# sail-sg/EditAnything

Measured on NVIDIA H100. Metric: 512x512 50-step SAM+ControlNet-inpaint images/sec; fused ControlNetx2+UNet+CFG+DDIM step ms, higher is better.
Workload: dtype fp16 storage / fp32 accumulate

## Files before the change

editanything_b200/csrc/ea_common.cuh:

```cuda
#pragma once
#include <cuda.h>
#include <cuda_fp16.h>
#include <cuda_bf16.h>
#include <cuda_runtime.h>
#include <stdint.h>
#include "ea_wgmma.cuh"

#ifdef EA_USE_BF16
typedef __nv_bfloat16 ea_half;
typedef __nv_bfloat162 ea_half2;
#define EA_TMAP_DTYPE CU_TENSOR_MAP_DATA_TYPE_BFLOAT16
__device__ __forceinline__ float ea_h2f(ea_half h) { return __bfloat162float(h); }
__device__ __forceinline__ ea_half ea_f2h(float f) { return __float2bfloat16_rn(f); }
__device__ __forceinline__ uint32_t ea_pack2(float a, float b) {
  __nv_bfloat162 v = __floats2bfloat162_rn(a, b);
  return *reinterpret_cast<uint32_t*>(&v);
}
__device__ __forceinline__ float2 ea_unpack2(uint32_t u) {
  __nv_bfloat162 v = *reinterpret_cast<__nv_bfloat162*>(&u);
  return __bfloat1622float2(v);
}
#else
typedef __half ea_half;
typedef __half2 ea_half2;
#define EA_TMAP_DTYPE CU_TENSOR_MAP_DATA_TYPE_FLOAT16
__device__ __forceinline__ float ea_h2f(ea_half h) { return __half2float(h); }
__device__ __forceinline__ ea_half ea_f2h(float f) { return __float2half_rn(f); }
__device__ __forceinline__ uint32_t ea_pack2(float a, float b) {
  __half2 v = __floats2half2_rn(a, b);
  return *reinterpret_cast<uint32_t*>(&v);
}
__device__ __forceinline__ float2 ea_unpack2(uint32_t u) {
  __half2 v = *reinterpret_cast<__half2*>(&u);
  return __half22float2(v);
}
#endif

namespace ea {

__device__ __forceinline__ uint32_t smem_u32(const void* p) {
  return static_cast<uint32_t>(__cvta_generic_to_shared(p));
}

__device__ __forceinline__ bool elect_one() {
  uint32_t pred = 0;
  asm volatile(
      "{\n\t.reg .pred P;\n\t"
      "elect.sync _|P, 0xffffffff;\n\t"
      "selp.b32 %0, 1, 0, P;\n\t}\n"
      : "=r"(pred));
  return pred != 0;
}

__device__ __forceinline__ void mbar_init(uint64_t* bar, uint32_t count) {
  asm volatile("mbarrier.init.shared::cta.b64 [%0], %1;" ::"r"(smem_u32(bar)), "r"(count));
}
__device__ __forceinline__ void fence_mbar_init() {
  asm volatile("fence.mbarrier_init.release.cluster;" ::: "memory");
}
__device__ __forceinline__ void fence_proxy_async() {
  asm volatile("fence.proxy.async.shared::cta;" ::: "memory");
}
__device__ __forceinline__ void mbar_expect_tx(uint64_t* bar, uint32_t bytes) {
  asm volatile("mbarrier.arrive.expect_tx.shared::cta.b64 _, [%0], %1;" ::"r"(smem_u32(bar)),
               "r"(bytes)
               : "memory");
}
__device__ __forceinline__ void mbar_arrive(uint64_t* bar) {
  asm volatile("mbarrier.arrive.shared::cta.b64 _, [%0];" ::"r"(smem_u32(bar)) : "memory");
}
__device__ __forceinline__ bool mbar_try_wait(uint64_t* bar, uint32_t parity) {
  uint32_t ok;
  asm volatile(
      "{\n\t.reg .pred P;\n\t"
      "mbarrier.try_wait.parity.shared::cta.b64 P, [%1], %2;\n\t"
      "selp.b32 %0, 1, 0, P;\n\t}\n"
      : "=r"(ok)
      : "r"(smem_u32(bar)), "r"(parity)
      : "memory");
  return ok != 0;
}
__device__ __forceinline__ void mbar_wait(uint64_t* bar, uint32_t parity) {
  uint32_t spins = 0;
  while (!mbar_try_wait(bar, parity)) {
    if (++spins > (1u << 28)) { asm volatile("trap;"); }
  }
}

__device__ __forceinline__ void tma_prefetch_desc(const CUtensorMap* m) {
  asm volatile("prefetch.tensormap [%0];" ::"l"(reinterpret_cast<uint64_t>(m)) : "memory");
}
__device__ __forceinline__ void tma_prefetch_l2_2d(const CUtensorMap* m, int c0, int c1) {
  asm volatile("cp.async.bulk.prefetch.tensor.2d.L2.global.tile [%0, {%1, %2}];" ::"l"(
                   reinterpret_cast<uint64_t>(m)),
               "r"(c0), "r"(c1)
               : "memory");
}
__device__ __forceinline__ void tma_load_2d(void* smem, const CUtensorMap* m, uint64_t* bar, int c0,
                                            int c1) {
  asm volatile(
      "cp.async.bulk.tensor.2d.shared::cluster.global.mbarrier::complete_tx::bytes [%0], [%1, {%3, "
      "%4}], [%2];" ::"r"(smem_u32(smem)),
      "l"(reinterpret_cast<uint64_t>(m)), "r"(smem_u32(bar)), "r"(c0), "r"(c1)
      : "memory");
}
__device__ __forceinline__ void tma_load_2d_hint(void* smem, const CUtensorMap* m, uint64_t* bar, int c0,
                                                 int c1, uint64_t policy) {
  if (policy == 0ull) {
    tma_load_2d(smem, m, bar, c0, c1);
    return;
  }
  asm volatile(
      "cp.async.bulk.tensor.2d.shared::cluster.global.mbarrier::complete_tx::bytes.L2::cache_hint [%0], [%1, {%3, "
      "%4}], [%2], %5;" ::"r"(smem_u32(smem)),
      "l"(reinterpret_cast<uint64_t>(m)), "r"(smem_u32(bar)), "r"(c0), "r"(c1), "l"(policy)
      : "memory");
}
__device__ __forceinline__ void tma_load_3d(void* smem, const CUtensorMap* m, uint64_t* bar, int c0,
                                            int c1, int c2) {
  asm volatile(
      "cp.async.bulk.tensor.3d.shared::cluster.global.mbarrier::complete_tx::bytes [%0], [%1, {%3, "
      "%4, %5}], [%2];" ::"r"(smem_u32(smem)),
      "l"(reinterpret_cast<uint64_t>(m)), "r"(smem_u32(bar)), "r"(c0), "r"(c1), "r"(c2)
      : "memory");
}
__device__ __forceinline__ void tma_load_4d(void* smem, const CUtensorMap* m, uint64_t* bar, int c0,
                                            int c1, int c2, int c3) {
  asm volatile(
      "cp.async.bulk.tensor.4d.shared::cluster.global.mbarrier::complete_tx::bytes [%0], [%1, {%3, "
      "%4, %5, %6}], [%2];" ::"r"(smem_u32(smem)),
      "l"(reinterpret_cast<uint64_t>(m)), "r"(smem_u32(bar)), "r"(c0), "r"(c1), "r"(c2), "r"(c3)
      : "memory");
}

__device__ __forceinline__ void wgmma_fence() { asm volatile("wgmma.fence.sync.aligned;" ::: "memory"); }
__device__ __forceinline__ void wgmma_commit() { asm volatile("wgmma.commit_group.sync.aligned;" ::: "memory"); }
template <int N>
__device__ __forceinline__ void wgmma_wait() {
  asm volatile("wgmma.wait_group.sync.aligned %0;" ::"n"(N) : "memory");
}
template <int R>
__device__ __forceinline__ void wgmma_fence_regs(float (&d)[R]) {
#pragma unroll
  for (int i = 0; i < R; ++i) asm volatile("" : "+f"(d[i])::"memory");
}

__device__ __forceinline__ uint64_t gmma_desc_k_sw128(uint32_t saddr, uint32_t sbo_bytes) {
  uint64_t d = 0;
  d |= (uint64_t)((saddr >> 4) & 0x3FFF);
  d |= (uint64_t)1 << 16;
  d |= (uint64_t)((sbo_bytes >> 4) & 0x3FFF) << 32;
  d |= (uint64_t)1 << 62;
  return d;
}
__device__ __forceinline__ uint64_t gmma_desc_mn_sw128(uint32_t saddr, uint32_t lbo_bytes,
                                                       uint32_t sbo_bytes) {
  uint64_t d = 0;
  d |= (uint64_t)((saddr >> 4) & 0x3FFF);
  d |= (uint64_t)((lbo_bytes >> 4) & 0x3FFF) << 16;
  d |= (uint64_t)((sbo_bytes >> 4) & 0x3FFF) << 32;
  d |= (uint64_t)1 << 62;
  return d;
}

__device__ __forceinline__ void pdl_wait() { asm volatile("griddepcontrol.wait;" ::: "memory"); }
__device__ __forceinline__ void pdl_launch_dependents() {
  asm volatile("griddepcontrol.launch_dependents;" ::: "memory");
}

__device__ __forceinline__ float mufu_ex2(float x) {
  float y;
  asm("ex2.approx.ftz.f32 %0, %1;" : "=f"(y) : "f"(x));
  return y;
}
__device__ __forceinline__ float mufu_rcp(float x) {
  float y;
  asm("rcp.approx.ftz.f32 %0, %1;" : "=f"(y) : "f"(x));
  return y;
}
__device__ __forceinline__ float silu_f(float x) {
  return x * mufu_rcp(1.0f + mufu_ex2(x * -1.4426950408889634f));
}
__device__ __forceinline__ float gelu_erf_f(float x) {
  const float z = fabsf(x) * 0.70710678118654752f;
  const float t = mufu_rcp(fmaf(0.3275911f, z, 1.0f));
  float poly = fmaf(1.061405429f, t, -1.453152027f);
  poly = fmaf(poly, t, 1.421413741f);
  poly = fmaf(poly, t, -0.284496736f);
  poly = fmaf(poly, t, 0.254829592f);
  const float e = fmaf(-poly * t, mufu_ex2(z * z * -1.4426950408889634f), 1.0f);
  return 0.5f * x * (1.0f + copysignf(e, x));
}
__device__ __forceinline__ float warp_sum(float v) {
#pragma unroll
  for (int o = 16; o > 0; o >>= 1) v += __shfl_xor_sync(0xffffffffu, v, o);
  return v;
}
__device__ __forceinline__ float warp_max(float v) {
#pragma unroll
  for (int o = 16; o > 0; o >>= 1) v = fmaxf(v, __shfl_xor_sync(0xffffffffu, v, o));
  return v;
}

}
```

editanything_b200/csrc/ea_gemm.cu:

```cuda
#include "ea_common.cuh"
#include "ea_internal.h"

namespace ea {

static constexpr int BM = 128;
static constexpr int BK = 64;
static constexpr int GEMM_THREADS = 288;
static constexpr int W_TMA = 8;
static constexpr int EPI_WARPS = 8, EPI_THREADS = 256;
static constexpr int GEMM_SMEM_RING = 216 * 1024;
__host__ __device__ constexpr int gemm_epi_bytes(int bn) { return BM * (bn + 4) * 4 + 2 * 4096 * EPI_WARPS; }
__host__ __device__ constexpr int gemm_region_bytes(int bn, int stages) {
  return stages * (BM * BK * 2 + bn * BK * 2) > gemm_epi_bytes(bn) ? stages * (BM * BK * 2 + bn * BK * 2)
                                                                    : gemm_epi_bytes(bn);
}

struct GemmKParams {
  int M, N;
  int mode;
  int nkb_main;
  int nkb_extra;
  int cin_blocks;
  int BN, stages;
  int H, W, Bsz;
  int bw, bh, bn;
  int tiles_w, tiles_h;
  const float* bias;
  const float* rowvec;
  int rows_per_batch;
  int rowvec_ld;
  const ea_half* residual;
  long long ldr;
  ea_half* out;
  long long ldo;
  ea_half* out2;
  long long ldo2;
  float* out_f32;
  int act;
  float out_scale;
  int accumulate;
  int splits;
  int kb_per_split;
  int no_spin;
  float* ws;
  int* cnt;
  float2* rowstats_out;
  const float2* ln_stats;
  const float* ln_g;
  int ln_parts;
  float ln_inv_c, ln_eps;
  const float* row_scale;
  const char* pf[EA_GEMM_MAX_PREFETCH];
  long long pf_bytes[EA_GEMM_MAX_PREFETCH];
  int pf_ctas;
  unsigned long long b_policy;
};

static constexpr int GEMM_MAX_GROUPS = 3;
struct GemmGroup {
  CUtensorMap tmA0, tmA1, tmA2, tmA3, tmAx, tmB;
  GemmKParams p;
};
template <int NG>
struct GemmLaunch {
  GemmGroup g[NG];
};

__device__ __forceinline__ void tile_origin(const GemmKParams& p, int tm, int& n0, int& h0,
                                            int& w0) {
  int per_blk = p.tiles_w * p.tiles_h;
  int nb = tm / per_blk;
  int r = tm - nb * per_blk;
  int th = r / p.tiles_w;
  n0 = nb * p.bn;
  h0 = th * p.bh;
  w0 = (r - th * p.tiles_w) * p.bw;
}

struct RowInfo {
  long long m;
  bool ok;
  int batch;
};

__device__ __forceinline__ RowInfo row_info(const GemmKParams& p, int tm, int r) {
  RowInfo ri;
  if (p.mode == EA_GEMM_LINEAR) {
    ri.m = (long long)tm * BM + r;
    ri.ok = ri.m < p.M;
    ri.batch = p.rows_per_batch > 0 ? (int)(ri.m / p.rows_per_batch) : 0;
  } else {
    int n0, h0, w0;
    tile_origin(p, tm, n0, h0, w0);
    int dn = r / (p.bw * p.bh);
    int rr = r - dn * (p.bw * p.bh);
    int dh = rr / p.bw;
    int dw = rr - dh * p.bw;
    int n = n0 + dn, h = h0 + dh, w = w0 + dw;
    ri.ok = (n < p.Bsz) && (h < p.H) && (w < p.W);
    ri.m = ((long long)n * p.H + h) * p.W + w;
    ri.batch = n;
  }
  return ri;
}

__device__ __forceinline__ void epi_bar_sync() { asm volatile("bar.sync 1, 256;" ::: "memory"); }

__device__ __forceinline__ int ld_acquire_gpu(const int* p) {
  int v;
  asm volatile("ld.acquire.gpu.global.s32 %0, [%1];" : "=r"(v) : "l"(p) : "memory");
  return v;
}

__device__ __forceinline__ void l2_prefetch_hint(const GemmKParams& p, int cta, int lane, int lane0) {
  if (cta >= p.pf_ctas || lane < lane0) return;
  const int nl = 32 - lane0;
#pragma unroll 1
  for (int i = 0; i < EA_GEMM_MAX_PREFETCH; ++i) {
    if (p.pf[i] == nullptr) continue;
    const long long nlines = p.pf_bytes[i] >> 7;
    const char* base = p.pf[i];
#pragma unroll 4
    for (long long c = (long long)cta * nl + (lane - lane0); c < nlines; c += (long long)p.pf_ctas * nl)
      asm volatile("prefetch.global.L2 [%0];" ::"l"(base + (c << 7)));
  }
}

__device__ __forceinline__ void ln_row_stats(const GemmKParams& p, long long m, float& ln_r, float& ln_nm) {
  float s = 0.f, q = 0.f;
  const float2* base = p.ln_stats + m;
  for (int j0 = 0; j0 < p.ln_parts; j0 += 16) {
    float2 v[16];
#pragma unroll
    for (int u = 0; u < 16; ++u)
      v[u] = (j0 + u < p.ln_parts) ? __ldcg(base + (size_t)(j0 + u) * p.M) : make_float2(0.f, 0.f);
#pragma unroll
    for (int u = 0; u < 16; ++u) {
      s += v[u].x;
      q += v[u].y;
    }
  }
  const float mu = s * p.ln_inv_c;
  ln_r = rsqrtf(fmaxf(q * p.ln_inv_c - mu * mu, 0.f) + p.ln_eps);
  ln_nm = -ln_r * mu;
}

__device__ __noinline__ float act_call(float x, int act) {
  return act == EA_ACT_SILU ? silu_f(x) : gelu_erf_f(x);
}

__device__ __forceinline__ void stage_put32(uint4* stg, int lane, int half, const uint4 (&o)[4]) {
#pragma unroll
  for (int q = 0; q < 4; ++q) stg[lane * 8 + ((half * 4 + q) ^ (lane & 7))] = o[q];
}
__device__ __forceinline__ void stage_flush(const uint4* stg, int lane, ea_half* out, long long ldo,
                                            ea_half* out2, long long ldo2, long long m_mine, bool ok_mine,
                                            int col0, int pieces, int n_limit, long long lin_m0, int M) {
  __syncwarp();
  const int piece = lane & 7, rsub = lane >> 3;
  const int col = col0 + piece * 8;
  const bool col_ok = piece < pieces && col < n_limit;
  uint4 val[8];
#pragma unroll
  for (int i = 0; i < 8; ++i) {
    const int row = i * 4 + rsub;
    val[i] = stg[row * 8 + (piece ^ (row & 7))];
  }
  if (lin_m0 >= 0) {
    const long long m0 = lin_m0 + rsub;
    ea_half* ptr = out + m0 * ldo + col;
    ea_half* ptr2 = out2 ? out2 + m0 * ldo2 + col : nullptr;
    const long long step = 4 * ldo, step2 = 4 * ldo2;
#pragma unroll
    for (int i = 0; i < 8; ++i) {
      if (col_ok && m0 + 4 * i < M) {
        *reinterpret_cast<uint4*>(ptr) = val[i];
        if (ptr2) *reinterpret_cast<uint4*>(ptr2) = val[i];
      }
      ptr += step;
      if (ptr2) ptr2 += step2;
    }
  } else {
#pragma unroll
    for (int i = 0; i < 8; ++i) {
      const int row = i * 4 + rsub;
      const long long m_r = __shfl_sync(0xffffffffu, m_mine, row);
      const int ok_r = __shfl_sync(0xffffffffu, (int)ok_mine, row);
      if (ok_r && col_ok) {
        *reinterpret_cast<uint4*>(out + m_r * ldo + col) = val[i];
        if (out2) *reinterpret_cast<uint4*>(out2 + m_r * ldo2 + col) = val[i];
      }
    }
  }
  __syncwarp();
}

__device__ __forceinline__ void stage_flush32(const uint4* stg, int lane, ea_half* out, long long ldo, int col0,
                                              int n_limit, long long lin_m0, int M) {
  __syncwarp();
  const int piece = lane & 3, rsub = lane >> 2;
  const int col = col0 + piece * 8;
  const bool col_ok = col < n_limit;
  uint4 val[4];
#pragma unroll
  for (int i = 0; i < 4; ++i) {
    const int row = i * 8 + rsub;
    val[i] = stg[row * 8 + (piece ^ (row & 7))];
  }
  const long long m0 = lin_m0 + rsub;
  ea_half* ptr = out + m0 * ldo + col;
  const long long step = 8 * ldo;
#pragma unroll
  for (int i = 0; i < 4; ++i) {
    if (col_ok && m0 + 8 * i < M) *reinterpret_cast<uint4*>(ptr) = val[i];
    ptr += step;
  }
  __syncwarp();
}

__device__ __forceinline__ void residual_load64(uint4 (&rr)[8], const ea_half* residual, long long ldr,
                                                int lane, long long m_mine, bool ok_mine, int col0,
                                                int cols_left, int n_limit, long long lin_m0, int M) {
  const int piece = lane & 7, rsub = lane >> 3;
  const int col = col0 + piece * 8;
#pragma unroll
  for (int i = 0; i < 8; ++i) {
    const int row = i * 4 + rsub;
    long long m_r;
    int ok_r;
    if (lin_m0 >= 0) {
      m_r = lin_m0 + row;
      ok_r = m_r < M;
    } else {
      m_r = __shfl_sync(0xffffffffu, m_mine, row);
      ok_r = __shfl_sync(0xffffffffu, (int)ok_mine, row);
    }
    rr[i] = (ok_r && piece * 8 < cols_left && col < n_limit)
                ? __ldg(reinterpret_cast<const uint4*>(residual + m_r * ldr + col))
                : make_uint4(0, 0, 0, 0);
  }
}

__device__ __forceinline__ void epilogue_geglu32(const float* cb, int half_bn, int c, float (&fx)[32],
                                                 float (&fg)[32], uint4 (&o)[4], bool ln, float ln_r,
                                                 float ln_nm) {
  uint32_t packed[16];
#pragma unroll
  for (int j = 0; j < 32; j += 4) {
    float4 bx = *reinterpret_cast<const float4*>(cb + c + j);
    float4 bg = *reinterpret_cast<const float4*>(cb + half_bn + c + j);
    if (ln) {
      const float4 gx = *reinterpret_cast<const float4*>(cb + 256 + c + j);
      const float4 gg = *reinterpret_cast<const float4*>(cb + 256 + half_bn + c + j);
      bx.x = fmaf(ln_nm, gx.x, bx.x); bx.y = fmaf(ln_nm, gx.y, bx.y); bx.z = fmaf(ln_nm, gx.z, bx.z); bx.w = fmaf(ln_nm, gx.w, bx.w);
      bg.x = fmaf(ln_nm, gg.x, bg.x); bg.y = fmaf(ln_nm, gg.y, bg.y); bg.z = fmaf(ln_nm, gg.z, bg.z); bg.w = fmaf(ln_nm, gg.w, bg.w);
    }
    const float x0 = fmaf(fx[j], ln_r, bx.x), x1 = fmaf(fx[j + 1], ln_r, bx.y);
    const float x2 = fmaf(fx[j + 2], ln_r, bx.z), x3 = fmaf(fx[j + 3], ln_r, bx.w);
    const float g0 = fmaf(fg[j], ln_r, bg.x), g1 = fmaf(fg[j + 1], ln_r, bg.y);
    const float g2 = fmaf(fg[j + 2], ln_r, bg.z), g3 = fmaf(fg[j + 3], ln_r, bg.w);
    packed[j >> 1] = ea_pack2(x0 * gelu_erf_f(g0), x1 * gelu_erf_f(g1));
    packed[(j >> 1) + 1] = ea_pack2(x2 * gelu_erf_f(g2), x3 * gelu_erf_f(g3));
  }
#pragma unroll
  for (int q = 0; q < 4; ++q)
    o[q] = make_uint4(packed[4 * q], packed[4 * q + 1], packed[4 * q + 2], packed[4 * q + 3]);
}

__device__ __forceinline__ void epilogue_geglu32_direct(const GemmKParams& p, const RowInfo& ri, int ncol0,
                                                        int half_bn, int c, float (&fx)[32],
                                                        float (&fg)[32]) {
  const int nout0 = (ncol0 >> 1) + c;
  if (!(ri.ok && nout0 < (p.N >> 1))) return;
  uint32_t packed[16];
#pragma unroll
  for (int j = 0; j < 32; j += 2) {
    float x0 = fx[j], x1 = fx[j + 1], g0 = fg[j], g1 = fg[j + 1];
    if (p.bias) {
      x0 += __ldg(p.bias + ncol0 + c + j);
      x1 += __ldg(p.bias + ncol0 + c + j + 1);
      g0 += __ldg(p.bias + ncol0 + half_bn + c + j);
      g1 += __ldg(p.bias + ncol0 + half_bn + c + j + 1);
    }
    packed[j >> 1] = ea_pack2(x0 * act_call(g0, EA_ACT_GELU), x1 * act_call(g1, EA_ACT_GELU));
  }
  uint4* dst = reinterpret_cast<uint4*>(p.out + ri.m * p.ldo + nout0);
#pragma unroll
  for (int q = 0; q < 4; ++q)
    dst[q] = make_uint4(packed[4 * q], packed[4 * q + 1], packed[4 * q + 2], packed[4 * q + 3]);
}

__device__ __forceinline__ void epilogue_chunk32(const GemmKParams& p, const RowInfo& ri,
                                                 int n_first, float (&f)[32]) {
  if (!(ri.ok && n_first < p.N)) return;
  const long long m = ri.m;
  if (p.bias) {
#pragma unroll
    for (int j = 0; j < 32; j += 4) {
      if (n_first + j < p.N) {
        float4 b = __ldg(reinterpret_cast<const float4*>(p.bias + n_first + j));
        f[j] += b.x; f[j + 1] += b.y; f[j + 2] += b.z; f[j + 3] += b.w;
      }
    }
  }
  if (p.rowvec) {
    const float* rv = p.rowvec + (long long)ri.batch * p.rowvec_ld + n_first;
#pragma unroll
    for (int j = 0; j < 32; j += 4) {
      if (n_first + j < p.N) {
        float4 b = __ldg(reinterpret_cast<const float4*>(rv + j));
        f[j] += b.x; f[j + 1] += b.y; f[j + 2] += b.z; f[j + 3] += b.w;
      }
    }
  }
  if (p.act == EA_ACT_SILU) {
#pragma unroll
    for (int j = 0; j < 32; ++j) f[j] = act_call(f[j], EA_ACT_SILU);
  } else if (p.act == EA_ACT_GELU) {
#pragma unroll
    for (int j = 0; j < 32; ++j) f[j] = act_call(f[j], EA_ACT_GELU);
  }
  if (p.out_scale != 1.0f) {
#pragma unroll
    for (int j = 0; j < 32; ++j) f[j] *= p.out_scale;
  }
  if (p.row_scale) {
    const float rs = __ldg(p.row_scale + m);
#pragma unroll
    for (int j = 0; j < 32; ++j) f[j] *= rs;
  }
  if (p.residual) {
    const uint4* rp = reinterpret_cast<const uint4*>(p.residual + m * p.ldr + n_first);
#pragma unroll
    for (int q = 0; q < 4; ++q) {
      if (n_first + q * 8 < p.N) {
        uint4 u = __ldg(rp + q);
        float2 a = ea_unpack2(u.x), b = ea_unpack2(u.y), cc = ea_unpack2(u.z), d = ea_unpack2(u.w);
        f[q * 8 + 0] += a.x; f[q * 8 + 1] += a.y; f[q * 8 + 2] += b.x; f[q * 8 + 3] += b.y;
        f[q * 8 + 4] += cc.x; f[q * 8 + 5] += cc.y; f[q * 8 + 6] += d.x; f[q * 8 + 7] += d.y;
      }
    }
  }
  if (p.out_f32) {
    float* dst = p.out_f32 + m * p.ldo + n_first;
#pragma unroll
    for (int j = 0; j < 32; j += 4) {
      if (n_first + j < p.N) {
        float4 o = make_float4(f[j], f[j + 1], f[j + 2], f[j + 3]);
        if (p.accumulate) {
          float4 old = *reinterpret_cast<float4*>(dst + j);
          o.x += old.x; o.y += old.y; o.z += old.z; o.w += old.w;
        }
        *reinterpret_cast<float4*>(dst + j) = o;
      }
    }
    return;
  }
  uint4* dst = reinterpret_cast<uint4*>(p.out + m * p.ldo + n_first);
  if (p.accumulate) {
#pragma unroll
    for (int q = 0; q < 4; ++q) {
      if (n_first + q * 8 < p.N) {
        uint4 u = dst[q];
        float2 a = ea_unpack2(u.x), b = ea_unpack2(u.y), cc = ea_unpack2(u.z), d = ea_unpack2(u.w);
        f[q * 8 + 0] += a.x; f[q * 8 + 1] += a.y; f[q * 8 + 2] += b.x; f[q * 8 + 3] += b.y;
        f[q * 8 + 4] += cc.x; f[q * 8 + 5] += cc.y; f[q * 8 + 6] += d.x; f[q * 8 + 7] += d.y;
      }
    }
  }
  uint4* dst2 = p.out2 ? reinterpret_cast<uint4*>(p.out2 + m * p.ldo2 + n_first) : nullptr;
#pragma unroll
  for (int q = 0; q < 4; ++q) {
    if (n_first + q * 8 < p.N) {
      uint4 o = make_uint4(ea_pack2(f[q * 8 + 0], f[q * 8 + 1]), ea_pack2(f[q * 8 + 2], f[q * 8 + 3]),
                           ea_pack2(f[q * 8 + 4], f[q * 8 + 5]), ea_pack2(f[q * 8 + 6], f[q * 8 + 7]));
      dst[q] = o;
      if (dst2) dst2[q] = o;
    }
  }
}


static int encode_2d(CUtensorMap* m, const void* base, uint64_t inner, uint64_t outer,
                     uint64_t row_stride_bytes, uint32_t box_inner, uint32_t box_outer) {
  cuuint64_t dims[2] = {inner, outer};
  cuuint64_t strides[1] = {row_stride_bytes};
  cuuint32_t box[2] = {box_inner, box_outer};
  cuuint32_t estr[2] = {1, 1};
  CUresult r = ea_tmap_encode()(m, EA_TMAP_DTYPE, 2, const_cast<void*>(base), dims, strides, box,
                                estr, CU_TENSOR_MAP_INTERLEAVE_NONE, CU_TENSOR_MAP_SWIZZLE_128B,
                                CU_TENSOR_MAP_L2_PROMOTION_L2_256B,
                                CU_TENSOR_MAP_FLOAT_OOB_FILL_NONE);
  return r == CUDA_SUCCESS ? 0 : (int)r;
}

static int encode_4d(CUtensorMap* m, const void* base, const uint64_t dims_[4],
                     const uint64_t strides_bytes[3], const uint32_t box_[4]) {
  cuuint64_t dims[4] = {dims_[0], dims_[1], dims_[2], dims_[3]};
  cuuint64_t strides[3] = {strides_bytes[0], strides_bytes[1], strides_bytes[2]};
  cuuint32_t box[4] = {box_[0], box_[1], box_[2], box_[3]};
  cuuint32_t estr[4] = {1, 1, 1, 1};
  CUresult r = ea_tmap_encode()(m, EA_TMAP_DTYPE, 4, const_cast<void*>(base), dims, strides, box,
                                estr, CU_TENSOR_MAP_INTERLEAVE_NONE, CU_TENSOR_MAP_SWIZZLE_128B,
                                CU_TENSOR_MAP_L2_PROMOTION_L2_256B,
                                CU_TENSOR_MAP_FLOAT_OOB_FILL_NONE);
  return r == CUDA_SUCCESS ? 0 : (int)r;
}

static void conv_geometry(int H, int W, int& bw, int& bh, int& bn) {
  bw = 1;
  while (bw * 2 <= W && bw * 2 <= 128 && (W % (bw * 2)) == 0) bw *= 2;
  bh = 1;
  while (bh * 2 <= H && bw * bh * 2 <= 128 && (H % (bh * 2)) == 0) bh *= 2;
  bn = 128 / (bw * bh);
}

__device__ __forceinline__ void acc_ld32(const float* accs, int ld, int r, int c, uint32_t (&v)[32]) {
  const float4* src = reinterpret_cast<const float4*>(accs + (size_t)r * ld + c);
#pragma unroll
  for (int j = 0; j < 8; ++j) {
    const float4 f = src[j];
    v[4 * j] = __float_as_uint(f.x); v[4 * j + 1] = __float_as_uint(f.y);
    v[4 * j + 2] = __float_as_uint(f.z); v[4 * j + 3] = __float_as_uint(f.w);
  }
}

#define EA_GEMM_TILE()                                                             \
  const int gi = NG == 1 ? 0 : tile / tiles_per_group;                             \
  const int gtile = NG == 1 ? tile : tile - gi * tiles_per_group;                  \
  const int zsplit = gtile / mn_tiles;                                             \
  const int mn = gtile - zsplit * mn_tiles;                                        \
  const GemmGroup& GG = L.g[gi];                                                   \
  const GemmKParams& p = GG.p;                                                     \
  const int tm = mn % m_tiles, tn = mn / m_tiles;                                  \
  const int kb0 = zsplit * p.kb_per_split;                                         \
  const int kb1 = min(nkb, kb0 + p.kb_per_split);

template <int BN, int NG>
__global__ void __launch_bounds__(GEMM_THREADS, 1)
ea_gemm_kernel(const __grid_constant__ GemmLaunch<NG> L, const int tiles_per_group, const int m_tiles,
               const int n_groups) {
  const GemmKParams& p0 = L.g[0].p;
  const int n_tiles = (p0.N + BN - 1) / BN;
  const int mn_tiles = m_tiles * n_tiles;
  const int num_tiles = tiles_per_group * (NG == 1 ? 1 : n_groups);
  const int nkb = p0.nkb_main + p0.nkb_extra;
  constexpr int a_bytes = BM * BK * 2;
  constexpr int stage_bytes = a_bytes + BN * BK * 2;
  constexpr int ACC_LD = BN + 4;
  extern __shared__ __align__(1024) uint8_t smem_raw[];
  uint8_t* smem = reinterpret_cast<uint8_t*>((reinterpret_cast<uintptr_t>(smem_raw) + 1023) &
                                             ~uintptr_t(1023));
  float* accs = reinterpret_cast<float*>(smem);
  uint8_t* stg_base = smem + BM * ACC_LD * 4;
  uint64_t* full_bar = reinterpret_cast<uint64_t*>(smem + gemm_region_bytes(BN, p0.stages));
  uint64_t* empty_bar = full_bar + p0.stages;
  uint64_t* epi_done = empty_bar + p0.stages;
  float* cb = reinterpret_cast<float*>(epi_done + 2);

  pdl_launch_dependents();
  const int warp = threadIdx.x >> 5;
  const int lane = threadIdx.x & 31;

  if (warp == W_TMA && lane == 0) {
    const int g0 = NG == 1 ? 0 : min((int)blockIdx.x / tiles_per_group, n_groups - 1);
    tma_prefetch_desc(&L.g[g0].tmA0);
    tma_prefetch_desc(&L.g[g0].tmB);
    if (p0.mode == EA_GEMM_CONV_S2 || p0.mode == EA_GEMM_CONV_S2A) {
      tma_prefetch_desc(&L.g[g0].tmA1);
      tma_prefetch_desc(&L.g[g0].tmA2);
      tma_prefetch_desc(&L.g[g0].tmA3);
    }
    if (p0.nkb_extra > 0) tma_prefetch_desc(&L.g[g0].tmAx);
  }
  if (warp == W_TMA) {
    for (int g = 0; g < (NG == 1 ? 1 : n_groups); ++g) l2_prefetch_hint(L.g[g].p, (int)blockIdx.x, lane, 2);
  }
  if (warp == W_TMA && lane == 1) {
    for (int s = 0; s < p0.stages; ++s) {
      mbar_init(&full_bar[s], 1);
      mbar_init(&empty_bar[s], EPI_WARPS);
    }
    mbar_init(epi_done, EPI_WARPS);
    fence_mbar_init();
  }
  __syncthreads();

  if (warp >= EPI_WARPS) {
    pdl_wait();
    if (lane != 0) return;
    int stage = 0;
    uint32_t phase = 0;
    uint8_t* sa = smem;
    int it = 0;
    for (int tile = blockIdx.x; tile < num_tiles; tile += gridDim.x, ++it) {
      EA_GEMM_TILE()
      const CUtensorMap& tmA0 = GG.tmA0;
      const CUtensorMap& tmA1 = GG.tmA1;
      const CUtensorMap& tmA2 = GG.tmA2;
      const CUtensorMap& tmA3 = GG.tmA3;
      const CUtensorMap& tmAx = GG.tmAx;
      const CUtensorMap& tmB = GG.tmB;
      if (it > 0) mbar_wait(epi_done, (uint32_t)((it - 1) & 1));
      const int bcol = tn * BN;
      if (p.mode == EA_GEMM_LINEAR) {
        const int arow = tm * BM;
        for (int kb = kb0; kb < kb1; ++kb) {
          mbar_wait(&empty_bar[stage], phase ^ 1u);
          mbar_expect_tx(&full_bar[stage], (uint32_t)stage_bytes);
          tma_load_2d(sa, &tmA0, &full_bar[stage], kb * BK, arow);
          tma_load_2d_hint(sa + a_bytes, &tmB, &full_bar[stage], kb * BK, bcol, p.b_policy);
          sa += stage_bytes;
          if (++stage == p.stages) { stage = 0; phase ^= 1u; sa = smem; }
        }
      } else {
        int n0, h0, w0;
        tile_origin(p, tm, n0, h0, w0);
        int tap = kb0 / p.cin_blocks;
        int c0 = (kb0 - tap * p.cin_blocks) * BK;
        int kh = tap / 3, kw = tap - kh * 3;
        const int cin = p.cin_blocks * BK;
        for (int kb = kb0; kb < kb1; ++kb) {
          mbar_wait(&empty_bar[stage], phase ^ 1u);
          mbar_expect_tx(&full_bar[stage], (uint32_t)stage_bytes);
          if (kb >= p.nkb_main) {
            tma_load_4d(sa, &tmAx, &full_bar[stage], (kb - p.nkb_main) * BK, w0, h0, n0);
          } else if (p.mode == EA_GEMM_CONV_S1) {
            tma_load_4d(sa, &tmA0, &full_bar[stage], c0, w0 + kw - 1, h0 + kh - 1, n0);
          } else {
            const bool asym = p.mode == EA_GEMM_CONV_S2A;
            const int ph = asym ? (kh == 1 ? 1 : 0) : (kh == 1 ? 0 : 1);
            const int dh = asym ? (kh == 2 ? 1 : 0) : (kh == 0 ? -1 : 0);
            const int pw = asym ? (kw == 1 ? 1 : 0) : (kw == 1 ? 0 : 1);
            const int dw = asym ? (kw == 2 ? 1 : 0) : (kw == 0 ? -1 : 0);
            const int sel = ph * 2 + pw;
            const CUtensorMap* m = sel == 0 ? &tmA0 : sel == 1 ? &tmA1 : sel == 2 ? &tmA2 : &tmA3;
            tma_load_4d(sa, m, &full_bar[stage], c0, w0 + dw, h0 + dh, n0);
          }
          tma_load_2d_hint(sa + a_bytes, &tmB, &full_bar[stage], kb * BK, bcol, p.b_policy);
          c0 += BK;
          if (c0 == cin) { c0 = 0; if (++kw == 3) { kw = 0; ++kh; } }
          sa += stage_bytes;
          if (++stage == p.stages) { stage = 0; phase ^= 1u; sa = smem; }
        }
      }
    }
    return;
  }

  pdl_wait();
  const int wg = warp >> 2;
  const int wq = warp & 3;
  const int r = wq * 32 + lane;
  const int et = threadIdx.x;
  constexpr int GSTEP = 128;
  uint4* stg = reinterpret_cast<uint4*>(stg_base + warp * 4096);
  uint4* stg2 = reinterpret_cast<uint4*>(stg_base + 4096 * EPI_WARPS + warp * 4096);
  const uint32_t smem0 = smem_u32(smem);
  int stage = 0;
  uint32_t phase = 0;
  int it = 0;
  for (int tile = blockIdx.x; tile < num_tiles; tile += gridDim.x, ++it) {
    EA_GEMM_TILE()
    const bool geglu = p.act == EA_ACT_GEGLU;
    const int half_bn = BN >> 1;
    const bool has_res = p.residual != nullptr;
    const RowInfo ri = row_info(p, tm, r);
    const int ncol0 = tn * BN;
    float* cbt = cb + (it & 1) * 512;
    const long long lin_m0 = p.mode == EA_GEMM_LINEAR ? (long long)tm * BM + wq * 32 : -1;
    const int b_first = row_info(p, tm, 0).batch, b_last = row_info(p, tm, BM - 1).batch;
    const bool fast = p.splits == 1 && !geglu && !p.out_f32 && !p.accumulate && !p.row_scale && (b_last - b_first) <= 1;
    uint4 rres[8];
    const bool ln = p.ln_stats != nullptr;
    float ln_r = 1.f, ln_nm = 0.f;
    if (ln && ri.ok) ln_row_stats(p, ri.m, ln_r, ln_nm);
    if (fast) {
      for (int i = et; i < BN; i += EPI_THREADS) {
        const int col = ncol0 + i;
        float v0 = 0.f, v1 = 0.f;
        if (col < p.N) {
          const float bsum = p.bias ? __ldg(p.bias + col) : 0.f;
          v0 = bsum + (p.rowvec ? __ldg(p.rowvec + (long long)b_first * p.rowvec_ld + col) : 0.f);
          v1 = ln ? __ldg(p.ln_g + col)
                  : bsum + (p.rowvec ? __ldg(p.rowvec + (long long)b_last * p.rowvec_ld + col) : 0.f);
        }
        cbt[i] = v0;
        cbt[256 + i] = v1;
      }
      if (has_res && wg * 64 < BN)
        residual_load64(rres, p.residual, p.ldr, lane, ri.m, ri.ok, ncol0 + wg * 64, BN - wg * 64, p.N, lin_m0, p.M);
    } else if (geglu && p.splits == 1) {
      for (int i = et; i < BN; i += EPI_THREADS) {
        const bool in = ncol0 + i < p.N;
        cbt[i] = (p.bias && in) ? __ldg(p.bias + ncol0 + i) : 0.f;
        if (ln) cbt[256 + i] = in ? __ldg(p.ln_g + ncol0 + i) : 0.f;
      }
    }

    {
      float acc[BN / 2];
#pragma unroll
      for (int i = 0; i < BN / 2; ++i) acc[i] = 0.f;
      int prev = -1;
      for (int kb = kb0; kb < kb1; ++kb) {
        mbar_wait(&full_bar[stage], phase);
        const uint32_t sa = smem0 + (uint32_t)(stage * stage_bytes);
        const uint64_t da = gmma_desc_k_sw128(sa + (uint32_t)(wg * 64 * 128), 1024);
        const uint64_t db = gmma_desc_k_sw128(sa + (uint32_t)a_bytes, 1024);
        wgmma_fence();
#pragma unroll
        for (int k = 0; k < 4; ++k) Wgmma<BN>::ss(acc, da + 2 * k, db + 2 * k, 1u);
        wgmma_commit();
        wgmma_wait<1>();
        if (prev >= 0) {
          __syncwarp();
          if (lane == 0) mbar_arrive(&empty_bar[prev]);
        }
        prev = stage;
        if (++stage == p.stages) { stage = 0; phase ^= 1u; }
      }
      wgmma_wait<0>();
      wgmma_fence_regs(acc);
      if (prev >= 0) {
        __syncwarp();
        if (lane == 0) mbar_arrive(&empty_bar[prev]);
      }
      epi_bar_sync();
      const int r0 = wg * 64 + wq * 16 + (lane >> 2);
      float* d0 = accs + (size_t)r0 * ACC_LD + 2 * (lane & 3);
#pragma unroll
      for (int j = 0; j < BN / 8; ++j) {
        *reinterpret_cast<float2*>(d0 + 8 * j) = make_float2(acc[4 * j], acc[4 * j + 1]);
        *reinterpret_cast<float2*>(d0 + 8 * ACC_LD + 8 * j) = make_float2(acc[4 * j + 2], acc[4 * j + 3]);
      }
    }
    epi_bar_sync();

    if (fast) {
      const float* cbr = cbt + ((!ln && ri.batch != b_first) ? 256 : 0);
      auto next_chunk = [&](int c) { return ((c & 32) == 0 && c + 32 < BN) ? c + 32 : (c & ~63) + GSTEP; };
      for (int c = wg * 64; c < BN; c = next_chunk(c)) {
        uint32_t v[32];
        acc_ld32(accs, ACC_LD, r, c, v);
        const int n_first = ncol0 + c;
        const int half = (c >> 5) & 1;
        if (has_res && half == 0) {
          const int piece = lane & 7, rsub = lane >> 3;
#pragma unroll
          for (int i = 0; i < 8; ++i) {
            const int row = i * 4 + rsub;
            stg2[row * 8 + (piece ^ (row & 7))] = rres[i];
          }
          __syncwarp();
          if (c + GSTEP < BN)
            residual_load64(rres, p.residual, p.ldr, lane, ri.m, ri.ok, n_first + GSTEP, BN - c - GSTEP, p.N, lin_m0, p.M);
        }
        float f[32];
        if (ln) {
#pragma unroll
          for (int j = 0; j < 32; j += 4) {
            const float4 b4 = *reinterpret_cast<const float4*>(cbt + c + j);
            const float4 g4 = *reinterpret_cast<const float4*>(cbt + 256 + c + j);
            f[j] = fmaf(__uint_as_float(v[j]), ln_r, fmaf(ln_nm, g4.x, b4.x));
            f[j + 1] = fmaf(__uint_as_float(v[j + 1]), ln_r, fmaf(ln_nm, g4.y, b4.y));
            f[j + 2] = fmaf(__uint_as_float(v[j + 2]), ln_r, fmaf(ln_nm, g4.z, b4.z));
            f[j + 3] = fmaf(__uint_as_float(v[j + 3]), ln_r, fmaf(ln_nm, g4.w, b4.w));
          }
        } else {
#pragma unroll
          for (int j = 0; j < 32; j += 4) {
            const float4 b4 = *reinterpret_cast<const float4*>(cbr + c + j);
            f[j] = __uint_as_float(v[j]) + b4.x;
            f[j + 1] = __uint_as_float(v[j + 1]) + b4.y;
            f[j + 2] = __uint_as_float(v[j + 2]) + b4.z;
            f[j + 3] = __uint_as_float(v[j + 3]) + b4.w;
          }
        }
        if (p.act == EA_ACT_SILU) {
#pragma unroll
          for (int j = 0; j < 32; ++j) f[j] = act_call(f[j], EA_ACT_SILU);
        } else if (p.act == EA_ACT_GELU) {
#pragma unroll
          for (int j = 0; j < 32; ++j) f[j] = gelu_erf_f(f[j]);
        }
        if (p.out_scale != 1.0f) {
#pragma unroll
          for (int j = 0; j < 32; ++j) f[j] *= p.out_scale;
        }
#pragma unroll
        for (int q = 0; q < 4; ++q) {
          const int slot = lane * 8 + ((half * 4 + q) ^ (lane & 7));
          if (has_res) {
            const uint4 rc = stg2[slot];
            const float2 a = ea_unpack2(rc.x), b = ea_unpack2(rc.y), cc = ea_unpack2(rc.z), d = ea_unpack2(rc.w);
            f[q * 8 + 0] += a.x; f[q * 8 + 1] += a.y; f[q * 8 + 2] += b.x; f[q * 8 + 3] += b.y;
            f[q * 8 + 4] += cc.x; f[q * 8 + 5] += cc.y; f[q * 8 + 6] += d.x; f[q * 8 + 7] += d.y;
          }
          stg[slot] = make_uint4(ea_pack2(f[q * 8 + 0], f[q * 8 + 1]), ea_pack2(f[q * 8 + 2], f[q * 8 + 3]),
                                 ea_pack2(f[q * 8 + 4], f[q * 8 + 5]), ea_pack2(f[q * 8 + 6], f[q * 8 + 7]));
        }
        if (p.rowstats_out) {
          float s0 = 0.f, s1 = 0.f, q0 = 0.f, q1 = 0.f;
#pragma unroll
          for (int j = 0; j < 32; j += 2) {
            s0 += f[j]; q0 = fmaf(f[j], f[j], q0);
            s1 += f[j + 1]; q1 = fmaf(f[j + 1], f[j + 1], q1);
          }
          if (ri.ok && n_first < p.N) p.rowstats_out[(size_t)(n_first >> 5) * p.M + ri.m] = make_float2(s0 + s1, q0 + q1);
        }
        if (half == 1 || c + 32 >= BN)
          stage_flush(stg, lane, p.out, p.ldo, p.out2, p.ldo2, ri.m, ri.ok, n_first - half * 32,
                      half == 1 ? 8 : 4, p.N, lin_m0, p.M);
      }
    } else if (p.splits == 1) {
      if (geglu) {
        for (int c = wg * 32; c < half_bn; c += 64) {
          uint32_t xv[32], gv[32];
          acc_ld32(accs, ACC_LD, r, c, xv);
          acc_ld32(accs, ACC_LD, r, half_bn + c, gv);
          float fx[32], fg[32];
#pragma unroll
          for (int j = 0; j < 32; ++j) { fx[j] = __uint_as_float(xv[j]); fg[j] = __uint_as_float(gv[j]); }
          uint4 o[4];
          epilogue_geglu32(cbt, half_bn, c, fx, fg, o, ln, ln_r, ln_nm);
          stage_put32(stg, lane, 0, o);
          if (lin_m0 >= 0)
            stage_flush32(stg, lane, p.out, p.ldo, (ncol0 >> 1) + c, p.N >> 1, lin_m0, p.M);
          else
            stage_flush(stg, lane, p.out, p.ldo, nullptr, 0, ri.m, ri.ok, (ncol0 >> 1) + c, 4, p.N >> 1, lin_m0, p.M);
        }
      } else {
        for (int c = wg * 32; c < BN; c += 64) {
          uint32_t v[32];
          acc_ld32(accs, ACC_LD, r, c, v);
          float f[32];
#pragma unroll
          for (int j = 0; j < 32; ++j) f[j] = __uint_as_float(v[j]);
          epilogue_chunk32(p, ri, ncol0 + c, f);
          __syncwarp();
        }
      }
    } else {
      const int tile_id = tn * m_tiles + tm;
      float* wtile = p.ws + (size_t)tile_id * p.splits * (BM * BN);
      float* mine = wtile + (size_t)zsplit * (BM * BN);
      for (int c = wg * 32; c < BN; c += 64) {
        uint32_t v[32];
        acc_ld32(accs, ACC_LD, r, c, v);
        float4* dst = reinterpret_cast<float4*>(mine + (size_t)r * BN + c);
#pragma unroll
        for (int j = 0; j < 8; ++j)
          __stcg(dst + j, make_float4(__uint_as_float(v[4 * j]), __uint_as_float(v[4 * j + 1]),
                                      __uint_as_float(v[4 * j + 2]), __uint_as_float(v[4 * j + 3])));
      }
      __threadfence();
      epi_bar_sync();
      int* cnt = p.cnt + 2 * tile_id;
      bool take_all = false;
      volatile int* flag = reinterpret_cast<volatile int*>(cbt);
      if (p.no_spin) {
        if (et == 0) *flag = atomicAdd(cnt, 1);
        epi_bar_sync();
        take_all = *flag == p.splits - 1;
        epi_bar_sync();
      } else {
        if (et == 0) {
          atomicAdd(cnt, 1);
          uint32_t spins = 0;
          while (ld_acquire_gpu(cnt) < p.splits) {
            __nanosleep(40);
            if (++spins > (1u << 24)) { asm volatile("trap;"); }
          }
        }
        epi_bar_sync();
      }
      __threadfence();
      if (!p.no_spin || take_all) {
        const int chunks = geglu ? (half_bn >> 5) : (BN >> 5);
        const int units = BM * chunks;
        const int u0 = take_all ? 0 : (int)(((long long)units * zsplit) / p.splits);
        const int u1 = take_all ? units : (int)(((long long)units * (zsplit + 1)) / p.splits);
        const int segs = geglu ? 2 : 1;
        const int ustride = segs * 32 + 4;
        float* stage_f = accs;
        const size_t split_stride = (size_t)BM * BN;
        for (int ub = u0; ub < u1; ub += EPI_THREADS) {
          const int nu = min(EPI_THREADS, u1 - ub);
          const int nvec4 = nu * segs * 8;
          for (int idx = et; idx < nvec4; idx += EPI_THREADS) {
            const int ul = idx / (segs * 8);
            const int rem = idx - ul * (segs * 8);
            const int seg = rem >> 3, q = rem & 7;
            const int u = ub + ul;
            const int rr = u & (BM - 1);
            const int c = ((u >> 7) << 5) + seg * half_bn * (geglu ? 1 : 0);
            const float4* src = reinterpret_cast<const float4*>(wtile + (size_t)rr * BN + c) + q;
            float4 acc = make_float4(0.f, 0.f, 0.f, 0.f);
            int sidx = 0;
            for (; sidx + 4 <= p.splits; sidx += 4) {
              float4 v0 = __ldcg(src + (size_t)(sidx + 0) * (split_stride >> 2));
              float4 v1 = __ldcg(src + (size_t)(sidx + 1) * (split_stride >> 2));
              float4 v2 = __ldcg(src + (size_t)(sidx + 2) * (split_stride >> 2));
              float4 v3 = __ldcg(src + (size_t)(sidx + 3) * (split_stride >> 2));
              acc.x += v0.x; acc.y += v0.y; acc.z += v0.z; acc.w += v0.w;
              acc.x += v1.x; acc.y += v1.y; acc.z += v1.z; acc.w += v1.w;
              acc.x += v2.x; acc.y += v2.y; acc.z += v2.z; acc.w += v2.w;
              acc.x += v3.x; acc.y += v3.y; acc.z += v3.z; acc.w += v3.w;
            }
            for (; sidx < p.splits; ++sidx) {
              float4 v0 = __ldcg(src + (size_t)sidx * (split_stride >> 2));
              acc.x += v0.x; acc.y += v0.y; acc.z += v0.z; acc.w += v0.w;
            }
            *reinterpret_cast<float4*>(stage_f + ul * ustride + seg * 32 + q * 4) = acc;
          }
          epi_bar_sync();
          if (et < nu) {
            const int u = ub + et;
            const int rr = u & (BM - 1);
            const int c = (u >> 7) << 5;
            RowInfo r2 = row_info(p, tm, rr);
            const float4* sp = reinterpret_cast<const float4*>(stage_f + et * ustride);
            float f[32];
#pragma unroll
            for (int j = 0; j < 8; ++j) {
              float4 v = sp[j];
              f[4 * j] = v.x; f[4 * j + 1] = v.y; f[4 * j + 2] = v.z; f[4 * j + 3] = v.w;
            }
            if (geglu) {
              float fg[32];
#pragma unroll
              for (int j = 0; j < 8; ++j) {
                float4 v = sp[8 + j];
                fg[4 * j] = v.x; fg[4 * j + 1] = v.y; fg[4 * j + 2] = v.z; fg[4 * j + 3] = v.w;
              }
              epilogue_geglu32_direct(p, r2, ncol0, half_bn, c, f, fg);
            } else {
              epilogue_chunk32(p, r2, ncol0 + c, f);
            }
          }
          epi_bar_sync();
        }
        epi_bar_sync();
        if (et == 0) {
          if (take_all) {
            cnt[0] = 0;
          } else {
            int old = atomicAdd(cnt + 1, 1);
            if (old == p.splits - 1) {
              cnt[0] = 0;
              cnt[1] = 0;
            }
          }
        }
      }
    }
    fence_proxy_async();
    __syncwarp();
    if (lane == 0) mbar_arrive(epi_done);
  }
}
#undef EA_GEMM_TILE

struct GemmPlan { int BN, stages, splits, kbps, occ; double cost; };

static constexpr double PL_LAT = 2100.0, PL_SM_CAP = 57.0, PL_L2 = 3000.0, PL_HBM = 1900.0;
static constexpr double PL_SPLIT_COL = 8.0, PL_SPLIT_FIX = 7000.0;
static constexpr double PL_START = 3800.0, PL_EPI = 50.0, PL_EPI_RES = 21.0;
static constexpr int GEMM_BN[3] = {128, 64, 32};

static GemmPlan plan_gemm(int mt, int N, int nkb, int act, long long ws_floats, int n_sm, bool has_res = false,
                          int groups = 1) {
  const double epi_col = (PL_EPI + (has_res ? PL_EPI_RES : 0.0)) * (act == EA_ACT_GEGLU ? 0.84 : 1.0);
  GemmPlan best = {0, 0, 1, nkb, 1, 1e30};
  for (int BN : GEMM_BN) {
    if (act == EA_ACT_GEGLU && BN != 128) continue;
    if (BN > 32 && N <= BN - 32) continue;
    const int nt = (N + BN - 1) / BN;
    const long long tiles = (long long)mt * nt * groups;
    const int stage_bytes = BM * BK * 2 + BN * BK * 2;
    int st = GEMM_SMEM_RING / stage_bytes;
    if (st > 8) st = 8;
    if (st > nkb) st = nkb < 2 ? 2 : nkb;
    const long long slots = n_sm;
    for (int pass = 0; pass < 2; ++pass) {
      int splits = 1, kbps = nkb;
      if (pass == 1) {
        if (tiles >= slots || nkb < 8) break;
        int s_max = (int)(slots / tiles);
        if (s_max > nkb / 4) s_max = nkb / 4;
        if (s_max < 2) break;
        kbps = (nkb + s_max - 1) / s_max;
        splits = (nkb + kbps - 1) / kbps;
        if (splits < 2) break;
        if (tiles > 2048 || tiles * splits * (long long)(BM * BN) > ws_floats) break;
      }
      const long long ctas = tiles * splits;
      const long long waves = (ctas + slots - 1) / slots;
      const long long conc = ctas < slots ? ctas : slots;
      const double t_mma = 4.0 * BN;
      const double t_sm = (double)stage_bytes / PL_SM_CAP;
      const double a_bytes = BM * BK * 2.0, b_bytes = BN * BK * 2.0;
      const double hbm_frac = 1.0 / (double)mt;
      const double t_chip = (double)conc * (a_bytes / PL_L2 + b_bytes * hbm_frac / PL_HBM +
                                            b_bytes * (1.0 - hbm_frac) / PL_L2);
      const double t_lat = PL_LAT / st;
      double t_kb = t_mma;
      if (t_sm > t_kb) t_kb = t_sm;
      if (t_chip > t_kb) t_kb = t_chip;
      if (t_lat > t_kb) t_kb = t_lat;
      double cost;
      if (splits == 1) {
        cost = (double)waves * (PL_START + kbps * t_kb + epi_col * BN);
      } else {
        cost = (double)waves * (PL_START + kbps * t_kb + PL_SPLIT_COL * BN) + PL_SPLIT_FIX +
               3.0 * (BM * BN * 4.0) / 25.0 + 150.0 * splits;
      }
      if (cost < best.cost) best = {BN, st, splits, kbps, 1, cost};
    }
  }
  return best;
}

static int sm_count() { return ea_sm_count(); }

}

using namespace ea;

extern "C" int ea_gemm_plan(int m_tiles, int N, int k_blocks, int act, long long workspace_bytes,
                            int n_sm, int* out5) {
  if (!out5 || m_tiles <= 0 || N <= 0 || k_blocks <= 0) return EA_ERR_ARG;
  const long long ws_floats = workspace_bytes > 65536 ? (workspace_bytes - 65536) / 4 : 0;
  GemmPlan pl = plan_gemm(m_tiles, N, k_blocks, act, ws_floats, n_sm > 0 ? n_sm : 132);
  out5[0] = pl.BN; out5[1] = pl.stages; out5[2] = pl.splits; out5[3] = pl.kbps;
  out5[4] = pl.occ;
  return pl.BN ? EA_OK : EA_ERR_SHAPE;
}

struct GemmShape {
  int m_tiles, nkb;
  long long Ktot;
  bool ln_any;
};

static int gemm_fill_group(const ea_gemm_args* a, GemmGroup& G, GemmShape& sh) {
  if (!a || !a->a || !a->w || (!a->out && !a->out_f32)) return EA_ERR_ARG;
  if (a->mode < 0 || a->mode > EA_GEMM_CONV_S2A) return EA_ERR_ARG;
  if (a->N <= 0 || a->M <= 0) return EA_ERR_ARG;
  if (a->N % 8 != 0) return EA_ERR_SHAPE;
  GemmKParams& p = G.p;
  memset(&p, 0, sizeof(p));
  p.M = a->M;
  p.N = a->N;
  p.mode = a->mode;
  p.bias = a->bias;
  p.rowvec = a->rowvec;
  p.rows_per_batch = a->rows_per_batch;
  p.rowvec_ld = a->rowvec_ld;
  p.residual = reinterpret_cast<const ea_half*>(a->residual);
  p.ldr = a->ldr;
  p.out = reinterpret_cast<ea_half*>(a->out);
  p.ldo = a->ldo;
  p.out2 = reinterpret_cast<ea_half*>(a->out2);
  p.ldo2 = a->ldo2;
  p.out_f32 = a->out_f32;
  p.act = a->act;
  p.out_scale = a->out_scale;
  p.accumulate = a->accumulate;
  p.row_scale = a->row_scale;
  for (int i = 0; i < EA_GEMM_MAX_PREFETCH; ++i) {
    p.pf[i] = reinterpret_cast<const char*>(a->prefetch[i]);
    p.pf_bytes[i] = a->prefetch[i] ? (a->prefetch_bytes[i] & ~15LL) : 0;
  }
  p.pf_ctas = 0;
  p.b_policy = 0x12F0000000000000ull;
  if (a->row_scale && (a->act == EA_ACT_GEGLU || a->rowstats_out || a->ln_stats)) return EA_ERR_ARG;
  sh.ln_any = a->rowstats_out || a->ln_stats;
  if (sh.ln_any) {
    if (a->mode != EA_GEMM_LINEAR || a->rowvec || a->out_f32 || a->accumulate) return EA_ERR_ARG;
    if (a->rowstats_out && (a->N % 32 != 0 || a->act == EA_ACT_GEGLU)) return EA_ERR_SHAPE;
    if (a->ln_stats && (!a->ln_g || a->ln_parts <= 0 || a->K != a->ln_parts * 32)) return EA_ERR_ARG;
    p.rowstats_out = reinterpret_cast<float2*>(a->rowstats_out);
    p.ln_stats = reinterpret_cast<const float2*>(a->ln_stats);
    p.ln_g = a->ln_g;
    p.ln_parts = a->ln_parts;
    p.ln_inv_c = a->ln_stats ? 1.0f / (float)a->K : 0.f;
    p.ln_eps = a->ln_eps;
  }
  if (p.ldo % 8 != 0 || (p.residual && p.ldr % 8 != 0) || (p.out2 && p.ldo2 % 8 != 0))
    return EA_ERR_SHAPE;

  CUtensorMap* tmA[4] = {&G.tmA0, &G.tmA1, &G.tmA2, &G.tmA3};
  if (a->mode == EA_GEMM_LINEAR) {
    if (a->K % 8 != 0 || a->lda % 8 != 0) return EA_ERR_SHAPE;
    p.nkb_main = (a->K + BK - 1) / BK;
    p.nkb_extra = 0;
    p.cin_blocks = 1;
    sh.m_tiles = (a->M + BM - 1) / BM;
    sh.Ktot = a->K;
    if (encode_2d(tmA[0], a->a, (uint64_t)a->K, (uint64_t)a->M, (uint64_t)a->lda * 2, BK, BM))
      return EA_ERR_TMAP;
    G.tmA1 = G.tmA2 = G.tmA3 = G.tmA0;
    G.tmAx = G.tmA0;
  } else {
    const int H = a->H, W = a->W, B = a->Bsz, C = a->Cin;
    if (C % 64 != 0 || H <= 0 || W <= 0 || B <= 0) return EA_ERR_SHAPE;
    if ((long long)B * H * W != a->M) return EA_ERR_SHAPE;
    p.H = H; p.W = W; p.Bsz = B;
    conv_geometry(H, W, p.bw, p.bh, p.bn);
    p.tiles_w = W / p.bw;
    p.tiles_h = H / p.bh;
    p.cin_blocks = C / 64;
    p.nkb_main = 9 * p.cin_blocks;
    p.nkb_extra = 0;
    sh.m_tiles = ((B + p.bn - 1) / p.bn) * p.tiles_w * p.tiles_h;
    sh.Ktot = 9LL * C;
    const long long lda = a->lda > 0 ? a->lda : C;
    uint32_t box[4] = {64, (uint32_t)p.bw, (uint32_t)p.bh, (uint32_t)p.bn};
    if (a->mode == EA_GEMM_CONV_S1) {
      uint64_t dims[4] = {(uint64_t)C, (uint64_t)W, (uint64_t)H, (uint64_t)B};
      uint64_t st[3] = {(uint64_t)lda * 2, (uint64_t)lda * W * 2, (uint64_t)lda * W * H * 2};
      if (encode_4d(tmA[0], a->a, dims, st, box)) return EA_ERR_TMAP;
      G.tmA1 = G.tmA2 = G.tmA3 = G.tmA0;
    } else {
      const int Hin = 2 * H, Win = 2 * W;
      for (int ph = 0; ph < 2; ++ph)
        for (int pw = 0; pw < 2; ++pw) {
          const ea_half* base =
              reinterpret_cast<const ea_half*>(a->a) + ((long long)ph * Win + pw) * lda;
          uint64_t dims[4] = {(uint64_t)C, (uint64_t)W, (uint64_t)H, (uint64_t)B};
          uint64_t st[3] = {(uint64_t)lda * 2 * 2, (uint64_t)lda * Win * 2 * 2,
                            (uint64_t)lda * Win * Hin * 2};
          if (encode_4d(tmA[ph * 2 + pw], base, dims, st, box)) return EA_ERR_TMAP;
        }
    }
    G.tmAx = G.tmA0;
    if (a->a_extra) {
      if (a->mode != EA_GEMM_CONV_S1 || a->Cin_extra % 64 != 0) return EA_ERR_SHAPE;
      const long long ldx = a->ld_extra > 0 ? a->ld_extra : a->Cin_extra;
      uint64_t dims[4] = {(uint64_t)a->Cin_extra, (uint64_t)W, (uint64_t)H, (uint64_t)B};
      uint64_t st[3] = {(uint64_t)ldx * 2, (uint64_t)ldx * W * 2, (uint64_t)ldx * W * H * 2};
      if (encode_4d(&G.tmAx, a->a_extra, dims, st, box)) return EA_ERR_TMAP;
      p.nkb_extra = a->Cin_extra / 64;
      sh.Ktot += a->Cin_extra;
    }
  }
  sh.nkb = p.nkb_main + p.nkb_extra;
  return EA_OK;
}

static bool gemm_same_problem(const ea_gemm_args* a, const ea_gemm_args* b) {
  return a->mode == b->mode && a->M == b->M && a->N == b->N && a->K == b->K && a->Bsz == b->Bsz && a->H == b->H &&
         a->W == b->W && a->Cin == b->Cin && a->Cin_extra == b->Cin_extra && (!a->a_extra) == (!b->a_extra) &&
         a->act == b->act && a->accumulate == b->accumulate && (!a->out_f32) == (!b->out_f32) &&
         (!a->row_scale) == (!b->row_scale) &&
         (!a->rowvec) == (!b->rowvec) && a->rows_per_batch == b->rows_per_batch &&
         (!a->rowstats_out) == (!b->rowstats_out) && (!a->ln_stats) == (!b->ln_stats) && a->ln_parts == b->ln_parts &&
         a->force_bn == b->force_bn && a->force_stages == b->force_stages && a->force_splits == b->force_splits &&
         a->force_2cta == b->force_2cta && a->no_spin == b->no_spin && a->force_persistent == b->force_persistent;
}

template <typename K>
static int set_max_smem(K kernel, int bytes, int& cached) {
  if (bytes > cached) {
    const cudaError_t e = cudaFuncSetAttribute(kernel, cudaFuncAttributeMaxDynamicSharedMemorySize, bytes);
    if (e != cudaSuccess) return ea_cuda_fail(e, "ea_gemm: cudaFuncSetAttribute(MaxDynamicSharedMemorySize)");
    cached = bytes;
  }
  return EA_OK;
}

template <int BN, int NG>
static cudaError_t launch_gemm(const GemmLaunch<NG>& L, int grid, int smem_bytes, int tiles_per_group, int m_tiles,
                               int n_groups, cudaStream_t stream, int& rc) {
  static int cache[EA_MAX_DEV];
  if ((rc = set_max_smem(ea_gemm_kernel<BN, NG>, smem_bytes, cache[ea_dev()]))) return cudaSuccess;
  return ea_launch(ea_gemm_kernel<BN, NG>, dim3((unsigned)grid), dim3(GEMM_THREADS), (size_t)smem_bytes, stream, L,
                   tiles_per_group, m_tiles, n_groups);
}

template <int NG>
static cudaError_t launch_gemm_bn(int BN, const GemmLaunch<NG>& L, int grid, int smem_bytes, int tiles_per_group,
                                  int m_tiles, int n_groups, cudaStream_t stream, int& rc) {
  switch (BN) {
    case 32: return launch_gemm<32, NG>(L, grid, smem_bytes, tiles_per_group, m_tiles, n_groups, stream, rc);
    case 64: return launch_gemm<64, NG>(L, grid, smem_bytes, tiles_per_group, m_tiles, n_groups, stream, rc);
    case 128: return launch_gemm<128, NG>(L, grid, smem_bytes, tiles_per_group, m_tiles, n_groups, stream, rc);
    default: return launch_gemm<256, NG>(L, grid, smem_bytes, tiles_per_group, m_tiles, n_groups, stream, rc);
  }
}

extern "C" int ea_gemm_grouped(const ea_gemm_args* args, int n_groups, void* stream_) {
  cudaStream_t stream = reinterpret_cast<cudaStream_t>(stream_);
  if (!args || n_groups < 1 || n_groups > GEMM_MAX_GROUPS) return EA_ERR_ARG;
  const ea_gemm_args* a = &args[0];
  static GemmLaunch<GEMM_MAX_GROUPS> L;
  GemmShape sh0;
  memset(&L, 0, sizeof(L));
  for (int g = 0; g < n_groups; ++g) {
    GemmShape shg;
    if (g > 0 && !gemm_same_problem(a, &args[g])) return EA_ERR_ARG;
    const int rc = gemm_fill_group(&args[g], L.g[g], g == 0 ? sh0 : shg);
    if (rc != EA_OK) return rc;
  }
  const int m_tiles = sh0.m_tiles, nkb = sh0.nkb;
  const bool ln_any = sh0.ln_any;
  const int G = n_groups;
  const long long ws_floats =
      (a->workspace && a->workspace_bytes > 65536 && !ln_any) ? (a->workspace_bytes - 65536) / 4 : 0;
  const bool persist = a->force_persistent > 0;
  const bool has_res = a->residual != nullptr;
  GemmPlan plan = plan_gemm(m_tiles, a->N, nkb, a->act, persist ? 0 : ws_floats, sm_count(), has_res, G);
  if (a->force_bn > 0 || a->force_stages > 0 || a->force_splits > 0) {
    if (a->force_bn > 0) plan.BN = a->force_bn;
    const int sb = BM * BK * 2 + plan.BN * BK * 2;
    if (a->force_bn > 0) plan.stages = plan.BN <= 128 ? 3 : 4;
    if (a->force_stages > 0) plan.stages = a->force_stages;
    if (plan.stages * sb > GEMM_SMEM_RING) plan.stages = GEMM_SMEM_RING / sb;
    if (plan.stages > nkb) plan.stages = nkb < 2 ? 2 : nkb;
    if (a->force_bn > 0 || a->force_splits > 0) { plan.splits = 1; plan.kbps = nkb; }
    if (a->force_splits > 1 && !persist) {
      plan.kbps = (nkb + a->force_splits - 1) / a->force_splits;
      plan.splits = (nkb + plan.kbps - 1) / plan.kbps;
    }
  }
  if (ln_any && plan.splits > 1) return EA_ERR_ARG;
  const int BN = plan.BN;
  if (BN != 32 && BN != 64 && BN != 128 && BN != 256) return EA_ERR_SHAPE;
  if (a->act == EA_ACT_GEGLU && (a->N % 128 != 0 || BN != 128)) return EA_ERR_SHAPE;
  const int n_tiles = (a->N + BN - 1) / BN;
  const long long tiles = (long long)m_tiles * n_tiles;
  if (plan.splits > 1 &&
      (!ws_floats || tiles * G > 8192 || tiles * G * plan.splits * (long long)(BM * BN) > ws_floats))
    return EA_ERR_SHAPE;
  if (plan.splits > 1 && !a->no_spin && tiles * G * plan.splits > (long long)sm_count()) return EA_ERR_SHAPE;

  int stages = plan.stages;
  if (stages > 8) stages = 8;
  if (stages < 2) stages = 2;
  const int smem_bytes = gemm_region_bytes(BN, stages) + (2 * stages + 2) * 8 + 2 * 2 * 256 * 4 + 1024;
  const long long tiles_per_group = tiles * plan.splits;
  for (int g = 0; g < G; ++g) {
    GemmKParams& p = L.g[g].p;
    const ea_gemm_args* ag = &args[g];
    p.BN = BN;
    p.stages = stages;
    p.splits = plan.splits;
    p.kb_per_split = plan.kbps;
    p.no_spin = a->no_spin;
    if (p.splits > 1) {
      p.cnt = reinterpret_cast<int*>(a->workspace) + 2 * g * tiles;
      p.ws = reinterpret_cast<float*>(reinterpret_cast<char*>(a->workspace) + 65536) +
             (size_t)g * tiles * p.splits * (BM * BN);
    }
    const long long ldw = ag->ldw > 0 ? ag->ldw : sh0.Ktot;
    if (ldw % 8 != 0) return EA_ERR_SHAPE;
    if (encode_2d(&L.g[g].tmB, ag->w, (uint64_t)sh0.Ktot, (uint64_t)ag->N, (uint64_t)ldw * 2, BK, (uint32_t)BN))
      return EA_ERR_TMAP;
  }
  if (m_tiles > 64)
    for (int g = 0; g < G; ++g) L.g[g].p.b_policy = 0ull;
  const long long total = tiles_per_group * G;
  const int grid = (int)(persist && total > sm_count() ? sm_count() : total);
  for (int g = 0; g < G; ++g)
    L.g[g].p.pf_ctas = grid < sm_count() ? grid : sm_count();

  cudaError_t le;
  int rc = EA_OK;
  if (G == 1) {
    GemmLaunch<1> L1;
    L1.g[0] = L.g[0];
    le = launch_gemm_bn<1>(BN, L1, grid, smem_bytes, (int)tiles_per_group, m_tiles, G, stream, rc);
  } else {
    le = launch_gemm_bn<GEMM_MAX_GROUPS>(BN, L, grid, smem_bytes, (int)tiles_per_group, m_tiles, G, stream, rc);
  }
  if (rc) return rc;
  ea_count_launch();
  if (le != cudaSuccess) return ea_cuda_fail(le, "ea_gemm: kernel launch");
  const cudaError_t ke = cudaGetLastError();
  return ke == cudaSuccess ? 0 : ea_cuda_fail(ke, "ea_gemm: after the kernel launch");
}

extern "C" int ea_gemm(const ea_gemm_args* a, void* stream) { return ea_gemm_grouped(a, 1, stream); }
```

Baseline: 1.610.

## Let one GEMM CTA compute two 128-row tiles sharing each B tile

Result: faster. 1.715, median of 6 (+6.5%).

```diff
diff --git a/editanything_b200/csrc/ea_common.cuh b/editanything_b200/csrc/ea_common.cuh
--- a/editanything_b200/csrc/ea_common.cuh
+++ b/editanything_b200/csrc/ea_common.cuh
@@ -144,6 +144,10 @@
 #pragma unroll
   for (int i = 0; i < R; ++i) asm volatile("" : "+f"(d[i])::"memory");
 }
+template <int R>
+__device__ __forceinline__ void setmaxnreg_dec() { asm volatile("setmaxnreg.dec.sync.aligned.u32 %0;" ::"n"(R)); }
+template <int R>
+__device__ __forceinline__ void setmaxnreg_inc() { asm volatile("setmaxnreg.inc.sync.aligned.u32 %0;" ::"n"(R)); }
 
 __device__ __forceinline__ uint64_t gmma_desc_k_sw128(uint32_t saddr, uint32_t sbo_bytes) {
   uint64_t d = 0;
diff --git a/editanything_b200/csrc/ea_gemm.cu b/editanything_b200/csrc/ea_gemm.cu
--- a/editanything_b200/csrc/ea_gemm.cu
+++ b/editanything_b200/csrc/ea_gemm.cu
@@ -5,15 +5,25 @@
 
 static constexpr int BM = 128;
 static constexpr int BK = 64;
-static constexpr int GEMM_THREADS = 288;
+static constexpr int GEMM_THREADS = 384;
 static constexpr int W_TMA = 8;
 static constexpr int EPI_WARPS = 8, EPI_THREADS = 256;
+static constexpr int PRODUCER_REGS = 56, CONSUMER_REGS = 224;
+static_assert(128 * PRODUCER_REGS + 256 * CONSUMER_REGS <= GEMM_THREADS * 168,
+              "setmaxnreg.inc can only take what .dec released from the CTA's launch allocation");
 static constexpr int GEMM_SMEM_RING = 216 * 1024;
-__host__ __device__ constexpr int gemm_epi_bytes(int bn) { return BM * (bn + 4) * 4 + 2 * 4096 * EPI_WARPS; }
-__host__ __device__ constexpr int gemm_region_bytes(int bn, int stages) {
-  return stages * (BM * BK * 2 + bn * BK * 2) > gemm_epi_bytes(bn) ? stages * (BM * BK * 2 + bn * BK * 2)
-                                                                    : gemm_epi_bytes(bn);
-}
+__host__ __device__ constexpr int gemm_stage_bytes(int bn, int rp) { return rp * BM * BK * 2 + bn * BK * 2; }
+__host__ __device__ constexpr int gemm_epi_bytes(int bn, int rp) {
+  return rp * BM * (bn + 4) * 4 + 2 * 4096 * EPI_WARPS;
+}
+__host__ __device__ constexpr int gemm_region_bytes(int bn, int stages, int rp) {
+  return stages * gemm_stage_bytes(bn, rp) > gemm_epi_bytes(bn, rp) ? stages * gemm_stage_bytes(bn, rp)
+                                                                    : gemm_epi_bytes(bn, rp);
+}
+static_assert(4 * gemm_stage_bytes(128, 2) <= GEMM_SMEM_RING, "RP = 2, BN = 128: four 48 KB stages fill the ring");
+static_assert(gemm_epi_bytes(128, 2) <= GEMM_SMEM_RING && gemm_epi_bytes(256, 1) <= GEMM_SMEM_RING,
+              "the staged accumulators and the store staging fit the ring");
+__host__ __device__ constexpr int gemm_cb_bytes(int rp) { return 2 * rp * 2 * 256 * 4; }
 
 struct GemmKParams {
   int M, N;
@@ -77,6 +87,11 @@
   w0 = (r - th * p.tiles_w) * p.bw;
 }
 
+__device__ __forceinline__ bool tile_valid(const GemmKParams& p, int tm) {
+  if (p.mode == EA_GEMM_LINEAR) return (long long)tm * BM < p.M;
+  return tm / (p.tiles_w * p.tiles_h) * p.bn < p.Bsz;
+}
+
 struct RowInfo {
   long long m;
   bool ok;
@@ -428,32 +443,34 @@
 #define EA_GEMM_TILE()                                                             \
   const int gi = NG == 1 ? 0 : tile / tiles_per_group;                             \
   const int gtile = NG == 1 ? tile : tile - gi * tiles_per_group;                  \
-  const int zsplit = gtile / mn_tiles;                                             \
-  const int mn = gtile - zsplit * mn_tiles;                                        \
+  const int zsplit = gtile / mn_items;                                             \
+  const int mn = gtile - zsplit * mn_items;                                        \
   const GemmGroup& GG = L.g[gi];                                                   \
   const GemmKParams& p = GG.p;                                                     \
-  const int tm = mn % m_tiles, tn = mn / m_tiles;                                  \
+  const int tp = mn % m_items, tn = mn / m_items;                                  \
+  const int tm0 = tp * RP;                                                         \
   const int kb0 = zsplit * p.kb_per_split;                                         \
   const int kb1 = min(nkb, kb0 + p.kb_per_split);
 
-template <int BN, int NG>
+template <int BN, int NG, int RP>
 __global__ void __launch_bounds__(GEMM_THREADS, 1)
-ea_gemm_kernel(const __grid_constant__ GemmLaunch<NG> L, const int tiles_per_group, const int m_tiles,
+ea_gemm_kernel(const __grid_constant__ GemmLaunch<NG> L, const int tiles_per_group, const int m_items,
                const int n_groups) {
+  static_assert(RP == 1 || (RP == 2 && BN <= 128), "two row tiles per CTA need BN <= 128 (registers)");
   const GemmKParams& p0 = L.g[0].p;
   const int n_tiles = (p0.N + BN - 1) / BN;
-  const int mn_tiles = m_tiles * n_tiles;
+  const int mn_items = m_items * n_tiles;
   const int num_tiles = tiles_per_group * (NG == 1 ? 1 : n_groups);
   const int nkb = p0.nkb_main + p0.nkb_extra;
   constexpr int a_bytes = BM * BK * 2;
-  constexpr int stage_bytes = a_bytes + BN * BK * 2;
+  constexpr int stage_bytes = gemm_stage_bytes(BN, RP);
   constexpr int ACC_LD = BN + 4;
   extern __shared__ __align__(1024) uint8_t smem_raw[];
   uint8_t* smem = reinterpret_cast<uint8_t*>((reinterpret_cast<uintptr_t>(smem_raw) + 1023) &
                                              ~uintptr_t(1023));
   float* accs = reinterpret_cast<float*>(smem);
-  uint8_t* stg_base = smem + BM * ACC_LD * 4;
-  uint64_t* full_bar = reinterpret_cast<uint64_t*>(smem + gemm_region_bytes(BN, p0.stages));
+  uint8_t* stg_base = smem + RP * BM * ACC_LD * 4;
+  uint64_t* full_bar = reinterpret_cast<uint64_t*>(smem + gemm_region_bytes(BN, p0.stages, RP));
   uint64_t* empty_bar = full_bar + p0.stages;
   uint64_t* epi_done = empty_bar + p0.stages;
   float* cb = reinterpret_cast<float*>(epi_done + 2);
@@ -487,8 +504,9 @@
   __syncthreads();
 
   if (warp >= EPI_WARPS) {
+    setmaxnreg_dec<PRODUCER_REGS>();
+    if (warp != W_TMA || lane != 0) return;
     pdl_wait();
-    if (lane != 0) return;
     int stage = 0;
     uint32_t phase = 0;
     uint8_t* sa = smem;
@@ -496,37 +514,40 @@
     for (int tile = blockIdx.x; tile < num_tiles; tile += gridDim.x, ++it) {
       EA_GEMM_TILE()
       const CUtensorMap& tmA0 = GG.tmA0;
-      const CUtensorMap& tmA1 = GG.tmA1;
-      const CUtensorMap& tmA2 = GG.tmA2;
-      const CUtensorMap& tmA3 = GG.tmA3;
       const CUtensorMap& tmAx = GG.tmAx;
       const CUtensorMap& tmB = GG.tmB;
       if (it > 0) mbar_wait(epi_done, (uint32_t)((it - 1) & 1));
       const int bcol = tn * BN;
+      const bool second = RP == 2 && tile_valid(p, tm0 + 1);
+      const uint32_t tx_bytes = (uint32_t)((second ? 2 : 1) * a_bytes + BN * BK * 2);
       if (p.mode == EA_GEMM_LINEAR) {
-        const int arow = tm * BM;
+        const int arow = tm0 * BM;
         for (int kb = kb0; kb < kb1; ++kb) {
           mbar_wait(&empty_bar[stage], phase ^ 1u);
-          mbar_expect_tx(&full_bar[stage], (uint32_t)stage_bytes);
+          mbar_expect_tx(&full_bar[stage], tx_bytes);
           tma_load_2d(sa, &tmA0, &full_bar[stage], kb * BK, arow);
-          tma_load_2d_hint(sa + a_bytes, &tmB, &full_bar[stage], kb * BK, bcol, p.b_policy);
+          if (second) tma_load_2d(sa + a_bytes, &tmA0, &full_bar[stage], kb * BK, arow + BM);
+          tma_load_2d_hint(sa + RP * a_bytes, &tmB, &full_bar[stage], kb * BK, bcol, p.b_policy);
           sa += stage_bytes;
           if (++stage == p.stages) { stage = 0; phase ^= 1u; sa = smem; }
         }
       } else {
-        int n0, h0, w0;
-        tile_origin(p, tm, n0, h0, w0);
+        int n0, h0, w0, n1 = 0, h1 = 0, w1 = 0;
+        tile_origin(p, tm0, n0, h0, w0);
+        if (second) tile_origin(p, tm0 + 1, n1, h1, w1);
         int tap = kb0 / p.cin_blocks;
         int c0 = (kb0 - tap * p.cin_blocks) * BK;
         int kh = tap / 3, kw = tap - kh * 3;
         const int cin = p.cin_blocks * BK;
         for (int kb = kb0; kb < kb1; ++kb) {
           mbar_wait(&empty_bar[stage], phase ^ 1u);
-          mbar_expect_tx(&full_bar[stage], (uint32_t)stage_bytes);
+          mbar_expect_tx(&full_bar[stage], tx_bytes);
           if (kb >= p.nkb_main) {
             tma_load_4d(sa, &tmAx, &full_bar[stage], (kb - p.nkb_main) * BK, w0, h0, n0);
+            if (second) tma_load_4d(sa + a_bytes, &tmAx, &full_bar[stage], (kb - p.nkb_main) * BK, w1, h1, n1);
           } else if (p.mode == EA_GEMM_CONV_S1) {
             tma_load_4d(sa, &tmA0, &full_bar[stage], c0, w0 + kw - 1, h0 + kh - 1, n0);
+            if (second) tma_load_4d(sa + a_bytes, &tmA0, &full_bar[stage], c0, w1 + kw - 1, h1 + kh - 1, n1);
           } else {
             const bool asym = p.mode == EA_GEMM_CONV_S2A;
             const int ph = asym ? (kh == 1 ? 1 : 0) : (kh == 1 ? 0 : 1);
@@ -534,10 +555,11 @@
             const int pw = asym ? (kw == 1 ? 1 : 0) : (kw == 1 ? 0 : 1);
             const int dw = asym ? (kw == 2 ? 1 : 0) : (kw == 0 ? -1 : 0);
             const int sel = ph * 2 + pw;
-            const CUtensorMap* m = sel == 0 ? &tmA0 : sel == 1 ? &tmA1 : sel == 2 ? &tmA2 : &tmA3;
+            const CUtensorMap* m = &tmA0 + sel;
             tma_load_4d(sa, m, &full_bar[stage], c0, w0 + dw, h0 + dh, n0);
+            if (second) tma_load_4d(sa + a_bytes, m, &full_bar[stage], c0, w1 + dw, h1 + dh, n1);
           }
-          tma_load_2d_hint(sa + a_bytes, &tmB, &full_bar[stage], kb * BK, bcol, p.b_policy);
+          tma_load_2d_hint(sa + RP * a_bytes, &tmB, &full_bar[stage], kb * BK, bcol, p.b_policy);
           c0 += BK;
           if (c0 == cin) { c0 = 0; if (++kw == 3) { kw = 0; ++kh; } }
           sa += stage_bytes;
@@ -548,12 +570,20 @@
     return;
   }
 
+  setmaxnreg_inc<CONSUMER_REGS>();
   pdl_wait();
   const int wg = warp >> 2;
   const int wq = warp & 3;
   const int r = wq * 32 + lane;
   const int et = threadIdx.x;
-  constexpr int GSTEP = 128;
+  const int sub = RP == 2 ? wg : 0;
+  const int ar = sub * BM + r;
+  constexpr int SUB_THREADS = EPI_THREADS / RP;
+  const int st_i = RP == 2 ? et & (SUB_THREADS - 1) : et;
+  const int c64 = RP == 2 ? 0 : wg * 64;
+  constexpr int GSTEP = RP == 2 ? 64 : 128;
+  const int c32 = RP == 2 ? 0 : wg * 32;
+  constexpr int CSTEP = RP == 2 ? 32 : 64;
   uint4* stg = reinterpret_cast<uint4*>(stg_base + warp * 4096);
   uint4* stg2 = reinterpret_cast<uint4*>(stg_base + 4096 * EPI_WARPS + warp * 4096);
   const uint32_t smem0 = smem_u32(smem);
@@ -562,21 +592,24 @@
   int it = 0;
   for (int tile = blockIdx.x; tile < num_tiles; tile += gridDim.x, ++it) {
     EA_GEMM_TILE()
+    const int tm = tm0 + sub;
+    const bool sub_ok = RP == 1 || tile_valid(p, tm);
     const bool geglu = p.act == EA_ACT_GEGLU;
     const int half_bn = BN >> 1;
     const bool has_res = p.residual != nullptr;
     const RowInfo ri = row_info(p, tm, r);
     const int ncol0 = tn * BN;
-    float* cbt = cb + (it & 1) * 512;
+    float* cbt = cb + ((it & 1) * RP + sub) * 512;
     const long long lin_m0 = p.mode == EA_GEMM_LINEAR ? (long long)tm * BM + wq * 32 : -1;
     const int b_first = row_info(p, tm, 0).batch, b_last = row_info(p, tm, BM - 1).batch;
-    const bool fast = p.splits == 1 && !geglu && !p.out_f32 && !p.accumulate && !p.row_scale && (b_last - b_first) <= 1;
+    const bool fast = sub_ok && p.splits == 1 && !geglu && !p.out_f32 && !p.accumulate && !p.row_scale &&
+                      (b_last - b_first) <= 1;
     uint4 rres[8];
     const bool ln = p.ln_stats != nullptr;
     float ln_r = 1.f, ln_nm = 0.f;
     if (ln && ri.ok) ln_row_stats(p, ri.m, ln_r, ln_nm);
     if (fast) {
-      for (int i = et; i < BN; i += EPI_THREADS) {
+      for (int i = st_i; i < BN; i += SUB_THREADS) {
         const int col = ncol0 + i;
         float v0 = 0.f, v1 = 0.f;
         if (col < p.N) {
@@ -588,10 +621,10 @@
         cbt[i] = v0;
         cbt[256 + i] = v1;
       }
-      if (has_res && wg * 64 < BN)
-        residual_load64(rres, p.residual, p.ldr, lane, ri.m, ri.ok, ncol0 + wg * 64, BN - wg * 64, p.N, lin_m0, p.M);
+      if (has_res && c64 < BN)
+        residual_load64(rres, p.residual, p.ldr, lane, ri.m, ri.ok, ncol0 + c64, BN - c64, p.N, lin_m0, p.M);
     } else if (geglu && p.splits == 1) {
-      for (int i = et; i < BN; i += EPI_THREADS) {
+      for (int i = st_i; i < BN; i += SUB_THREADS) {
         const bool in = ncol0 + i < p.N;
         cbt[i] = (p.bias && in) ? __ldg(p.bias + ncol0 + i) : 0.f;
         if (ln) cbt[256 + i] = in ? __ldg(p.ln_g + ncol0 + i) : 0.f;
@@ -599,18 +632,24 @@
     }
 
     {
-      float acc[BN / 2];
-#pragma unroll
-      for (int i = 0; i < BN / 2; ++i) acc[i] = 0.f;
+      float acc[RP][BN / 2];
+#pragma unroll
+      for (int h = 0; h < RP; ++h)
+#pragma unroll
+        for (int i = 0; i < BN / 2; ++i) acc[h][i] = 0.f;
+      const uint32_t a_off = RP == 2 ? (uint32_t)(wg * a_bytes) : (uint32_t)(wg * 64 * 128);
       int prev = -1;
       for (int kb = kb0; kb < kb1; ++kb) {
         mbar_wait(&full_bar[stage], phase);
         const uint32_t sa = smem0 + (uint32_t)(stage * stage_bytes);
-        const uint64_t da = gmma_desc_k_sw128(sa + (uint32_t)(wg * 64 * 128), 1024);
-        const uint64_t db = gmma_desc_k_sw128(sa + (uint32_t)a_bytes, 1024);
+        const uint64_t db = gmma_desc_k_sw128(sa + (uint32_t)(RP * a_bytes), 1024);
         wgmma_fence();
 #pragma unroll
-        for (int k = 0; k < 4; ++k) Wgmma<BN>::ss(acc, da + 2 * k, db + 2 * k, 1u);
+        for (int h = 0; h < RP; ++h) {
+          const uint64_t da = gmma_desc_k_sw128(sa + a_off + (uint32_t)(h * 64 * 128), 1024);
+#pragma unroll
+          for (int k = 0; k < 4; ++k) Wgmma<BN>::ss(acc[h], da + 2 * k, db + 2 * k, 1u);
+        }
         wgmma_commit();
         wgmma_wait<1>();
         if (prev >= 0) {
@@ -621,18 +660,22 @@
         if (++stage == p.stages) { stage = 0; phase ^= 1u; }
       }
       wgmma_wait<0>();
-      wgmma_fence_regs(acc);
+#pragma unroll
+      for (int h = 0; h < RP; ++h) wgmma_fence_regs(acc[h]);
       if (prev >= 0) {
         __syncwarp();
         if (lane == 0) mbar_arrive(&empty_bar[prev]);
       }
       epi_bar_sync();
-      const int r0 = wg * 64 + wq * 16 + (lane >> 2);
-      float* d0 = accs + (size_t)r0 * ACC_LD + 2 * (lane & 3);
-#pragma unroll
-      for (int j = 0; j < BN / 8; ++j) {
-        *reinterpret_cast<float2*>(d0 + 8 * j) = make_float2(acc[4 * j], acc[4 * j + 1]);
-        *reinterpret_cast<float2*>(d0 + 8 * ACC_LD + 8 * j) = make_float2(acc[4 * j + 2], acc[4 * j + 3]);
+#pragma unroll
+      for (int h = 0; h < RP; ++h) {
+        const int r0 = (RP == 2 ? wg * BM + h * 64 : wg * 64) + wq * 16 + (lane >> 2);
+        float* d0 = accs + (size_t)r0 * ACC_LD + 2 * (lane & 3);
+#pragma unroll
+        for (int j = 0; j < BN / 8; ++j) {
+          *reinterpret_cast<float2*>(d0 + 8 * j) = make_float2(acc[h][4 * j], acc[h][4 * j + 1]);
+          *reinterpret_cast<float2*>(d0 + 8 * ACC_LD + 8 * j) = make_float2(acc[h][4 * j + 2], acc[h][4 * j + 3]);
+        }
       }
     }
     epi_bar_sync();
@@ -640,9 +683,9 @@
     if (fast) {
       const float* cbr = cbt + ((!ln && ri.batch != b_first) ? 256 : 0);
       auto next_chunk = [&](int c) { return ((c & 32) == 0 && c + 32 < BN) ? c + 32 : (c & ~63) + GSTEP; };
-      for (int c = wg * 64; c < BN; c = next_chunk(c)) {
+      for (int c = c64; c < BN; c = next_chunk(c)) {
         uint32_t v[32];
-        acc_ld32(accs, ACC_LD, r, c, v);
+        acc_ld32(accs, ACC_LD, ar, c, v);
         const int n_first = ncol0 + c;
         const int half = (c >> 5) & 1;
         if (has_res && half == 0) {
@@ -715,10 +758,10 @@
       }
     } else if (p.splits == 1) {
       if (geglu) {
-        for (int c = wg * 32; c < half_bn; c += 64) {
+        for (int c = c32; c < half_bn; c += CSTEP) {
           uint32_t xv[32], gv[32];
-          acc_ld32(accs, ACC_LD, r, c, xv);
-          acc_ld32(accs, ACC_LD, r, half_bn + c, gv);
+          acc_ld32(accs, ACC_LD, ar, c, xv);
+          acc_ld32(accs, ACC_LD, ar, half_bn + c, gv);
           float fx[32], fg[32];
 #pragma unroll
           for (int j = 0; j < 32; ++j) { fx[j] = __uint_as_float(xv[j]); fg[j] = __uint_as_float(gv[j]); }
@@ -731,9 +774,9 @@
             stage_flush(stg, lane, p.out, p.ldo, nullptr, 0, ri.m, ri.ok, (ncol0 >> 1) + c, 4, p.N >> 1, lin_m0, p.M);
         }
       } else {
-        for (int c = wg * 32; c < BN; c += 64) {
+        for (int c = c32; c < BN; c += CSTEP) {
           uint32_t v[32];
-          acc_ld32(accs, ACC_LD, r, c, v);
+          acc_ld32(accs, ACC_LD, ar, c, v);
           float f[32];
 #pragma unroll
           for (int j = 0; j < 32; ++j) f[j] = __uint_as_float(v[j]);
@@ -742,13 +785,14 @@
         }
       }
     } else {
-      const int tile_id = tn * m_tiles + tm;
-      float* wtile = p.ws + (size_t)tile_id * p.splits * (BM * BN);
-      float* mine = wtile + (size_t)zsplit * (BM * BN);
-      for (int c = wg * 32; c < BN; c += 64) {
+      constexpr int RB = RP * BM;
+      const int tile_id = tn * m_items + tp;
+      float* wtile = p.ws + (size_t)tile_id * p.splits * (RB * BN);
+      float* mine = wtile + (size_t)zsplit * (RB * BN);
+      for (int c = c32; c < BN; c += CSTEP) {
         uint32_t v[32];
-        acc_ld32(accs, ACC_LD, r, c, v);
-        float4* dst = reinterpret_cast<float4*>(mine + (size_t)r * BN + c);
+        acc_ld32(accs, ACC_LD, ar, c, v);
+        float4* dst = reinterpret_cast<float4*>(mine + (size_t)ar * BN + c);
 #pragma unroll
         for (int j = 0; j < 8; ++j)
           __stcg(dst + j, make_float4(__uint_as_float(v[4 * j]), __uint_as_float(v[4 * j + 1]),
@@ -758,7 +802,7 @@
       epi_bar_sync();
       int* cnt = p.cnt + 2 * tile_id;
       bool take_all = false;
-      volatile int* flag = reinterpret_cast<volatile int*>(cbt);
+      volatile int* flag = reinterpret_cast<volatile int*>(cb + (it & 1) * RP * 512);
       if (p.no_spin) {
         if (et == 0) *flag = atomicAdd(cnt, 1);
         epi_bar_sync();
@@ -778,13 +822,13 @@
       __threadfence();
       if (!p.no_spin || take_all) {
         const int chunks = geglu ? (half_bn >> 5) : (BN >> 5);
-        const int units = BM * chunks;
+        const int units = RB * chunks;
         const int u0 = take_all ? 0 : (int)(((long long)units * zsplit) / p.splits);
         const int u1 = take_all ? units : (int)(((long long)units * (zsplit + 1)) / p.splits);
         const int segs = geglu ? 2 : 1;
         const int ustride = segs * 32 + 4;
         float* stage_f = accs;
-        const size_t split_stride = (size_t)BM * BN;
+        const size_t split_stride = (size_t)RB * BN;
         for (int ub = u0; ub < u1; ub += EPI_THREADS) {
           const int nu = min(EPI_THREADS, u1 - ub);
           const int nvec4 = nu * segs * 8;
@@ -793,8 +837,8 @@
             const int rem = idx - ul * (segs * 8);
             const int seg = rem >> 3, q = rem & 7;
             const int u = ub + ul;
-            const int rr = u & (BM - 1);
-            const int c = ((u >> 7) << 5) + seg * half_bn * (geglu ? 1 : 0);
+            const int rr = u & (RB - 1);
+            const int c = ((u / RB) << 5) + seg * half_bn * (geglu ? 1 : 0);
             const float4* src = reinterpret_cast<const float4*>(wtile + (size_t)rr * BN + c) + q;
             float4 acc = make_float4(0.f, 0.f, 0.f, 0.f);
             int sidx = 0;
@@ -817,9 +861,9 @@
           epi_bar_sync();
           if (et < nu) {
             const int u = ub + et;
-            const int rr = u & (BM - 1);
-            const int c = (u >> 7) << 5;
-            RowInfo r2 = row_info(p, tm, rr);
+            const int rr = u & (RB - 1);
+            const int c = (u / RB) << 5;
+            RowInfo r2 = row_info(p, tm0 + rr / BM, rr & (BM - 1));
             const float4* sp = reinterpret_cast<const float4*>(stage_f + et * ustride);
             float f[32];
 #pragma unroll
@@ -862,7 +906,7 @@
 }
 #undef EA_GEMM_TILE
 
-struct GemmPlan { int BN, stages, splits, kbps, occ; double cost; };
+struct GemmPlan { int BN, stages, splits, kbps, occ, rp; double cost; };
 
 static constexpr double PL_LAT = 2100.0, PL_SM_CAP = 57.0, PL_L2 = 3000.0, PL_HBM = 1900.0;
 static constexpr double PL_SPLIT_COL = 8.0, PL_SPLIT_FIX = 7000.0;
@@ -870,53 +914,59 @@
 static constexpr int GEMM_BN[3] = {128, 64, 32};
 
 static GemmPlan plan_gemm(int mt, int N, int nkb, int act, long long ws_floats, int n_sm, bool has_res = false,
-                          int groups = 1) {
+                          int groups = 1, int force_rp = 0) {
   const double epi_col = (PL_EPI + (has_res ? PL_EPI_RES : 0.0)) * (act == EA_ACT_GEGLU ? 0.84 : 1.0);
-  GemmPlan best = {0, 0, 1, nkb, 1, 1e30};
-  for (int BN : GEMM_BN) {
-    if (act == EA_ACT_GEGLU && BN != 128) continue;
-    if (BN > 32 && N <= BN - 32) continue;
-    const int nt = (N + BN - 1) / BN;
-    const long long tiles = (long long)mt * nt * groups;
-    const int stage_bytes = BM * BK * 2 + BN * BK * 2;
-    int st = GEMM_SMEM_RING / stage_bytes;
-    if (st > 8) st = 8;
-    if (st > nkb) st = nkb < 2 ? 2 : nkb;
-    const long long slots = n_sm;
-    for (int pass = 0; pass < 2; ++pass) {
-      int splits = 1, kbps = nkb;
-      if (pass == 1) {
-        if (tiles >= slots || nkb < 8) break;
-        int s_max = (int)(slots / tiles);
-        if (s_max > nkb / 4) s_max = nkb / 4;
-        if (s_max < 2) break;
-        kbps = (nkb + s_max - 1) / s_max;
-        splits = (nkb + kbps - 1) / kbps;
-        if (splits < 2) break;
-        if (tiles > 2048 || tiles * splits * (long long)(BM * BN) > ws_floats) break;
-      }
-      const long long ctas = tiles * splits;
-      const long long waves = (ctas + slots - 1) / slots;
-      const long long conc = ctas < slots ? ctas : slots;
-      const double t_mma = 4.0 * BN;
-      const double t_sm = (double)stage_bytes / PL_SM_CAP;
-      const double a_bytes = BM * BK * 2.0, b_bytes = BN * BK * 2.0;
-      const double hbm_frac = 1.0 / (double)mt;
-      const double t_chip = (double)conc * (a_bytes / PL_L2 + b_bytes * hbm_frac / PL_HBM +
-                                            b_bytes * (1.0 - hbm_frac) / PL_L2);
-      const double t_lat = PL_LAT / st;
-      double t_kb = t_mma;
-      if (t_sm > t_kb) t_kb = t_sm;
-      if (t_chip > t_kb) t_kb = t_chip;
-      if (t_lat > t_kb) t_kb = t_lat;
-      double cost;
-      if (splits == 1) {
-        cost = (double)waves * (PL_START + kbps * t_kb + epi_col * BN);
-      } else {
-        cost = (double)waves * (PL_START + kbps * t_kb + PL_SPLIT_COL * BN) + PL_SPLIT_FIX +
-               3.0 * (BM * BN * 4.0) / 25.0 + 150.0 * splits;
-      }
-      if (cost < best.cost) best = {BN, st, splits, kbps, 1, cost};
+  GemmPlan best = {0, 0, 1, nkb, 1, 1, 1e30};
+  for (int rp = 1; rp <= 2; ++rp) {
+    if (force_rp > 0 && rp != force_rp) continue;
+    if (force_rp == 0 && rp == 2 && mt < 2) continue;
+    const int mi = (mt + rp - 1) / rp;
+    for (int BN : GEMM_BN) {
+      if (act == EA_ACT_GEGLU && BN != 128) continue;
+      if (BN > 32 && N <= BN - 32) continue;
+      const int nt = (N + BN - 1) / BN;
+      const long long tiles = (long long)mi * nt * groups;
+      const int stage_bytes = gemm_stage_bytes(BN, rp);
+      int st = GEMM_SMEM_RING / stage_bytes;
+      if (st > 8) st = 8;
+      if (st > nkb) st = nkb < 2 ? 2 : nkb;
+      const long long slots = n_sm;
+      if (force_rp == 0 && rp == 2 && (long long)mt * nt * groups <= slots) continue;
+      for (int pass = 0; pass < (rp == 1 ? 2 : 1); ++pass) {
+        int splits = 1, kbps = nkb;
+        if (pass == 1) {
+          if (tiles >= slots || nkb < 8) break;
+          int s_max = (int)(slots / tiles);
+          if (s_max > nkb / 4) s_max = nkb / 4;
+          if (s_max < 2) break;
+          kbps = (nkb + s_max - 1) / s_max;
+          splits = (nkb + kbps - 1) / kbps;
+          if (splits < 2) break;
+          if (tiles > 2048 || tiles * splits * (long long)(BM * BN) > ws_floats) break;
+        }
+        const long long ctas = tiles * splits;
+        const long long waves = (ctas + slots - 1) / slots;
+        const long long conc = ctas < slots ? ctas : slots;
+        const double t_mma = 4.0 * BN * rp;
+        const double t_sm = (double)stage_bytes / PL_SM_CAP;
+        const double a_bytes = rp * BM * BK * 2.0, b_bytes = BN * BK * 2.0;
+        const double hbm_frac = 1.0 / (double)mi;
+        const double t_chip = (double)conc * (a_bytes / PL_L2 + b_bytes * hbm_frac / PL_HBM +
+                                              b_bytes * (1.0 - hbm_frac) / PL_L2);
+        const double t_lat = PL_LAT / st;
+        double t_kb = t_mma;
+        if (t_sm > t_kb) t_kb = t_sm;
+        if (t_chip > t_kb) t_kb = t_chip;
+        if (t_lat > t_kb) t_kb = t_lat;
+        double cost;
+        if (splits == 1) {
+          cost = (double)waves * (PL_START + kbps * t_kb + epi_col * BN * rp);
+        } else {
+          cost = (double)waves * (PL_START + kbps * t_kb + PL_SPLIT_COL * BN) + PL_SPLIT_FIX +
+                 3.0 * (BM * BN * 4.0) / 25.0 + 150.0 * splits;
+        }
+        if (cost < best.cost) best = {BN, st, splits, kbps, 1, rp, cost};
+      }
     }
   }
   return best;
@@ -1071,23 +1121,30 @@
   return EA_OK;
 }
 
-template <int BN, int NG>
-static cudaError_t launch_gemm(const GemmLaunch<NG>& L, int grid, int smem_bytes, int tiles_per_group, int m_tiles,
+template <int BN, int NG, int RP>
+static cudaError_t launch_gemm(const GemmLaunch<NG>& L, int grid, int smem_bytes, int tiles_per_group, int m_items,
                                int n_groups, cudaStream_t stream, int& rc) {
   static int cache[EA_MAX_DEV];
-  if ((rc = set_max_smem(ea_gemm_kernel<BN, NG>, smem_bytes, cache[ea_dev()]))) return cudaSuccess;
-  return ea_launch(ea_gemm_kernel<BN, NG>, dim3((unsigned)grid), dim3(GEMM_THREADS), (size_t)smem_bytes, stream, L,
-                   tiles_per_group, m_tiles, n_groups);
+  if ((rc = set_max_smem(ea_gemm_kernel<BN, NG, RP>, smem_bytes, cache[ea_dev()]))) return cudaSuccess;
+  return ea_launch(ea_gemm_kernel<BN, NG, RP>, dim3((unsigned)grid), dim3(GEMM_THREADS), (size_t)smem_bytes, stream,
+                   L, tiles_per_group, m_items, n_groups);
 }
 
 template <int NG>
-static cudaError_t launch_gemm_bn(int BN, const GemmLaunch<NG>& L, int grid, int smem_bytes, int tiles_per_group,
-                                  int m_tiles, int n_groups, cudaStream_t stream, int& rc) {
+static cudaError_t launch_gemm_bn(int BN, int rp, const GemmLaunch<NG>& L, int grid, int smem_bytes,
+                                  int tiles_per_group, int m_items, int n_groups, cudaStream_t stream, int& rc) {
+  if (rp == 2) {
+    switch (BN) {
+      case 32: return launch_gemm<32, NG, 2>(L, grid, smem_bytes, tiles_per_group, m_items, n_groups, stream, rc);
+      case 64: return launch_gemm<64, NG, 2>(L, grid, smem_bytes, tiles_per_group, m_items, n_groups, stream, rc);
+      default: return launch_gemm<128, NG, 2>(L, grid, smem_bytes, tiles_per_group, m_items, n_groups, stream, rc);
+    }
+  }
   switch (BN) {
-    case 32: return launch_gemm<32, NG>(L, grid, smem_bytes, tiles_per_group, m_tiles, n_groups, stream, rc);
-    case 64: return launch_gemm<64, NG>(L, grid, smem_bytes, tiles_per_group, m_tiles, n_groups, stream, rc);
-    case 128: return launch_gemm<128, NG>(L, grid, smem_bytes, tiles_per_group, m_tiles, n_groups, stream, rc);
-    default: return launch_gemm<256, NG>(L, grid, smem_bytes, tiles_per_group, m_tiles, n_groups, stream, rc);
+    case 32: return launch_gemm<32, NG, 1>(L, grid, smem_bytes, tiles_per_group, m_items, n_groups, stream, rc);
+    case 64: return launch_gemm<64, NG, 1>(L, grid, smem_bytes, tiles_per_group, m_items, n_groups, stream, rc);
+    case 128: return launch_gemm<128, NG, 1>(L, grid, smem_bytes, tiles_per_group, m_items, n_groups, stream, rc);
+    default: return launch_gemm<256, NG, 1>(L, grid, smem_bytes, tiles_per_group, m_items, n_groups, stream, rc);
   }
 }
 
@@ -1111,10 +1168,16 @@
       (a->workspace && a->workspace_bytes > 65536 && !ln_any) ? (a->workspace_bytes - 65536) / 4 : 0;
   const bool persist = a->force_persistent > 0;
   const bool has_res = a->residual != nullptr;
-  GemmPlan plan = plan_gemm(m_tiles, a->N, nkb, a->act, persist ? 0 : ws_floats, sm_count(), has_res, G);
+  const int force_rp = a->force_2cta > 0 ? 2 : a->force_2cta < 0 ? 1 : 0;
+  GemmPlan plan =
+      plan_gemm(m_tiles, a->N, nkb, a->act, persist ? 0 : ws_floats, sm_count(), has_res, G, force_rp);
+  if (a->force_bn > 256 - 128 * (plan.rp - 1)) {
+    if (force_rp == 2) return EA_ERR_SHAPE;
+    plan.rp = 1;
+  }
   if (a->force_bn > 0 || a->force_stages > 0 || a->force_splits > 0) {
     if (a->force_bn > 0) plan.BN = a->force_bn;
-    const int sb = BM * BK * 2 + plan.BN * BK * 2;
+    const int sb = gemm_stage_bytes(plan.BN, plan.rp);
     if (a->force_bn > 0) plan.stages = plan.BN <= 128 ? 3 : 4;
     if (a->force_stages > 0) plan.stages = a->force_stages;
     if (plan.stages * sb > GEMM_SMEM_RING) plan.stages = GEMM_SMEM_RING / sb;
@@ -1126,20 +1189,21 @@
     }
   }
   if (ln_any && plan.splits > 1) return EA_ERR_ARG;
-  const int BN = plan.BN;
+  const int BN = plan.BN, RP = plan.rp;
   if (BN != 32 && BN != 64 && BN != 128 && BN != 256) return EA_ERR_SHAPE;
   if (a->act == EA_ACT_GEGLU && (a->N % 128 != 0 || BN != 128)) return EA_ERR_SHAPE;
   const int n_tiles = (a->N + BN - 1) / BN;
-  const long long tiles = (long long)m_tiles * n_tiles;
+  const int m_items = (m_tiles + RP - 1) / RP;
+  const long long tiles = (long long)m_items * n_tiles;
   if (plan.splits > 1 &&
-      (!ws_floats || tiles * G > 8192 || tiles * G * plan.splits * (long long)(BM * BN) > ws_floats))
+      (!ws_floats || tiles * G > 8192 || tiles * G * plan.splits * (long long)(RP * BM * BN) > ws_floats))
     return EA_ERR_SHAPE;
   if (plan.splits > 1 && !a->no_spin && tiles * G * plan.splits > (long long)sm_count()) return EA_ERR_SHAPE;
 
   int stages = plan.stages;
   if (stages > 8) stages = 8;
   if (stages < 2) stages = 2;
-  const int smem_bytes = gemm_region_bytes(BN, stages) + (2 * stages + 2) * 8 + 2 * 2 * 256 * 4 + 1024;
+  const int smem_bytes = gemm_region_bytes(BN, stages, RP) + (2 * stages + 2) * 8 + gemm_cb_bytes(RP) + 1024;
   const long long tiles_per_group = tiles * plan.splits;
   for (int g = 0; g < G; ++g) {
     GemmKParams& p = L.g[g].p;
@@ -1152,7 +1216,7 @@
     if (p.splits > 1) {
       p.cnt = reinterpret_cast<int*>(a->workspace) + 2 * g * tiles;
       p.ws = reinterpret_cast<float*>(reinterpret_cast<char*>(a->workspace) + 65536) +
-             (size_t)g * tiles * p.splits * (BM * BN);
+             (size_t)g * tiles * p.splits * (RP * BM * BN);
     }
     const long long ldw = ag->ldw > 0 ? ag->ldw : sh0.Ktot;
     if (ldw % 8 != 0) return EA_ERR_SHAPE;
@@ -1171,9 +1235,9 @@
   if (G == 1) {
     GemmLaunch<1> L1;
     L1.g[0] = L.g[0];
-    le = launch_gemm_bn<1>(BN, L1, grid, smem_bytes, (int)tiles_per_group, m_tiles, G, stream, rc);
+    le = launch_gemm_bn<1>(BN, RP, L1, grid, smem_bytes, (int)tiles_per_group, m_items, G, stream, rc);
   } else {
-    le = launch_gemm_bn<GEMM_MAX_GROUPS>(BN, L, grid, smem_bytes, (int)tiles_per_group, m_tiles, G, stream, rc);
+    le = launch_gemm_bn<GEMM_MAX_GROUPS>(BN, RP, L, grid, smem_bytes, (int)tiles_per_group, m_items, G, stream, rc);
   }
   if (rc) return rc;
   ea_count_launch();
```
